# zjsun1017/CUDA-Go-ICP

Measured on AMD Instinct MI355X. Metric: bnb_cube_bounds_per_s, higher is better.
Workload: dtype f32; 1 GPU; bunny_goicp.toml (BASELINE configs[1]): N=30379 source, M=35947 target, DT 300^3, subsample 1.0; dt_layout=bricked4x4x4, exchange=local min

## Files before the change

cuda-go-icp_amd/binding.py:

```python
import ctypes as C
import os
import subprocess

HERE = os.path.dirname(os.path.abspath(__file__))
_LIB = None

OK = 0
STATUS = {-1: "GOICP_ERR_INVALID", -2: "GOICP_ERR_IO", -3: "GOICP_ERR_CONFIG", -4: "GOICP_ERR_NO_DEVICE",
          -5: "GOICP_ERR_DEVICE", -6: "GOICP_ERR_INTERNAL", -7: "GOICP_ERR_TIMEOUT", -8: "GOICP_ERR_PEER"}
PATH_MAX = 1024


class GoicpError(RuntimeError):
    def __init__(self, code, msg):
        super().__init__("%s: %s" % (STATUS.get(code, str(code)), msg))
        self.code = code


class CConfig(C.Structure):
    _fields_ = [("mode", C.c_int32), ("trim", C.c_int32), ("subsample", C.c_float), ("mse_threshold", C.c_float),
                ("resize", C.c_float), ("target", C.c_char * PATH_MAX), ("source", C.c_char * PATH_MAX),
                ("output", C.c_char * PATH_MAX), ("visualization", C.c_char * PATH_MAX),
                ("viz_theta", C.c_float), ("viz_phi", C.c_float), ("viz_spin_after_finish", C.c_int32),
                ("rot_min", C.c_float * 3), ("rot_max", C.c_float * 3), ("rot_search_depth", C.c_int32),
                ("trans_min", C.c_float * 3), ("trans_max", C.c_float * 3), ("trans_search_depth", C.c_int32),
                ("description", C.c_char * PATH_MAX), ("has_rotation_range", C.c_int32), ("has_translation_range", C.c_int32)]


class CParams(C.Structure):
    _fields_ = [("dt_size", C.c_int32), ("dt_expand", C.c_double), ("mse_threshold", C.c_float),
                ("dt_layout", C.c_int32), ("device", C.c_int32), ("trans_batch", C.c_int32),
                ("wide_children", C.c_int32), ("icp_max_iter", C.c_int32), ("verbose", C.c_int32),
                ("morton_sort", C.c_int32), ("rot_batch", C.c_int32), ("kd_gpu_build", C.c_int32), ("trim_fraction", C.c_float),
                ("use_rot_range", C.c_int32), ("use_trans_range", C.c_int32), ("rot_min", C.c_float * 3), ("rot_max", C.c_float * 3),
                ("trans_min", C.c_float * 3), ("trans_max", C.c_float * 3), ("rot_search_depth", C.c_int32), ("trans_search_depth", C.c_int32),
                ("icp_fused", C.c_int32), ("bounds_fp16", C.c_int32), ("icp_nn_cache", C.c_int32), ("flow", C.c_int32), ("adaptive_k", C.c_int32), ("queue_cap", C.c_int32), ("device_queues", C.c_int32),
                ("lds_tiles", C.c_int32), ("tile_spread_vox", C.c_float), ("tile_min", C.c_int32), ("stale_widen", C.c_int32), ("ub_tiebreak", C.c_int32), ("icp_point_seed", C.c_int32), ("ub_share", C.c_float), ("twin_fusion", C.c_int32), ("sort_items", C.c_int32), ("stale_compact", C.c_int32), ("stream_priority", C.c_int32), ("lanes", C.c_int32), ("lane_min_searches", C.c_int32),
                ("bounds_order", C.c_int32), ("bounds_order_min_groups", C.c_int32), ("bounds_order_max_runs", C.c_int32), ("bounds_order_cell", C.c_float), ("bounds_order_reprobe", C.c_int32),
                ("bounds_balance", C.c_int32), ("bounds_balance_a", C.c_float)]


class CCube(C.Structure):
    _fields_ = [("tx", C.c_float), ("ty", C.c_float), ("tz", C.c_float), ("delta", C.c_float),
                ("coeff", C.c_float), ("rot", C.c_int32)]


class CCounters(C.Structure):
    _fields_ = [(n, C.c_int64) for n in ("rot_pops", "trans_pops", "cubes", "inner_calls", "icp_runs", "icp_iters",
                                         "bounds_launches", "queue_fallbacks", "tile_expansions", "lane_batches")]


class CResult(C.Structure):
    _fields_ = [("optR", C.c_float * 9), ("optT", C.c_float * 3), ("curR", C.c_float * 9), ("curT", C.c_float * 3),
                ("best_sse", C.c_float), ("finished", C.c_int32), ("counters", CCounters),
                ("dt_build_ms", C.c_double), ("register_ms", C.c_double)]


class CStepStatus(C.Structure):
    _fields_ = [("finished", C.c_int32), ("early_exit", C.c_int32), ("best_sse", C.c_float),
                ("frontier_lb", C.c_float), ("rot_pops", C.c_int64)]


ALLREDUCE_FN = C.CFUNCTYPE(C.c_int, C.c_void_p, C.POINTER(C.c_uint64), C.c_size_t)
BCAST_FN = C.CFUNCTYPE(C.c_int, C.c_void_p, C.c_void_p, C.c_size_t, C.c_int32)


class CCommOps(C.Structure):
    _fields_ = [("ctx", C.c_void_p), ("rank", C.c_int32), ("world", C.c_int32), ("allreduce_min_u64", ALLREDUCE_FN), ("bcast", BCAST_FN)]


class CShardStats(C.Structure):
    _fields_ = [(n, C.c_int64) for n in ("steps", "exchanges", "broadcasts", "donations", "donated_cubes", "steps_idle")] + \
               [("wait_ms", C.c_double), ("step_ms", C.c_double), ("best_sse", C.c_float), ("failed_rank", C.c_int32)]


class CIcpShardStats(C.Structure):
    _fields_ = [(n, C.c_int32) for n in ("rank", "world", "block_begin", "block_end", "blocks", "sliced")] + \
               [(n, C.c_int64) for n in ("queries", "runs", "passes", "collectives")] + \
               [("sum_wait_ms", C.c_double), ("round_trip_ms", C.c_double)]


class CIcpOptions(C.Structure):
    _fields_ = [("metric", C.c_int32), ("normal_k", C.c_int32)]


class CIcpGate(C.Structure):
    _fields_ = [("max_corr_dist", C.c_float), ("min_inliers", C.c_int32), ("capped_walk", C.c_int32)]


class CIcpRobust(C.Structure):
    _fields_ = [("kernel", C.c_int32), ("scale", C.c_float)]


class CSourceFilter(C.Structure):
    _fields_ = [("voxel", C.c_float), ("radius", C.c_float), ("min_neighbors", C.c_int32)]


class CSourcePipeline(C.Structure):
    _fields_ = [("voxel", C.c_float), ("stat_neighbors", C.c_int32), ("stat_std_ratio", C.c_float), ("radius", C.c_float), ("min_neighbors", C.c_int32)]


class CClusterSelect(C.Structure):
    _fields_ = [("radius", C.c_float), ("min_neighbors", C.c_int32), ("min_size", C.c_int32), ("max_clusters", C.c_int32)]


class CPlaneSelect(C.Structure):
    _fields_ = [("distance", C.c_float), ("iterations", C.c_int32), ("refine", C.c_int32), ("max_planes", C.c_int32), ("min_inliers", C.c_int32),
                ("seed", C.c_uint64)]


class CPlane(C.Structure):
    _fields_ = [("normal", C.c_float * 3), ("point", C.c_float * 3), ("d", C.c_float), ("inliers", C.c_int32), ("hypothesis", C.c_int32),
                ("refined", C.c_int32)]


PLANE_MAX_ITERATIONS = 65536
PLANE_MAX_PLANES = 8


class CRansacPoseSelect(C.Structure):
    _fields_ = [("distance", C.c_float), ("iterations", C.c_int32), ("refine", C.c_int32), ("max_poses", C.c_int32), ("min_inliers", C.c_int32),
                ("edge_similarity", C.c_float), ("seed", C.c_uint64)]


class CRansacPose(C.Structure):
    _fields_ = [("R", C.c_float * 9), ("t", C.c_float * 3), ("inliers", C.c_int32), ("hypothesis", C.c_int32), ("refined", C.c_int32)]


RANSAC_POSE_MAX_ITERATIONS = 1 << 20
RANSAC_POSE_MAX_POSES = 64


class CPoseInfoOptions(C.Structure):
    _fields_ = [("metric", C.c_int32), ("use_pivot", C.c_int32), ("pivot", C.c_double * 3), ("rank_tol", C.c_double)]


class CPoseInfo(C.Structure):
    _fields_ = [("information", C.c_double * 36), ("gradient", C.c_double * 6), ("covariance", C.c_double * 36), ("eigenvalues", C.c_double * 6),
                ("eigenvectors", C.c_double * 36), ("pivot", C.c_double * 3), ("weight_sum", C.c_double), ("cost", C.c_double), ("sse", C.c_double),
                ("sigma2", C.c_double), ("inliers", C.c_int64), ("rank", C.c_int32), ("metric", C.c_int32), ("dof_nonpositive", C.c_int32)]


class CShardOptions(C.Structure):
    _fields_ = [("rot_pops_per_step", C.c_int32), ("rebalance", C.c_int32), ("stale_exchange", C.c_int32), ("ramp_to", C.c_int32)]


_fpp = C.POINTER(C.c_float)
ENG_BEGIN_FN = C.CFUNCTYPE(C.c_int, C.c_void_p, C.c_int32, C.c_int32)
ENG_STEP_FN = C.CFUNCTYPE(C.c_int, C.c_void_p, C.c_int32, C.POINTER(CStepStatus))
ENG_POSE_FN = C.CFUNCTYPE(C.c_int, C.c_void_p, _fpp, _fpp, _fpp)
ENG_OFFER_FN = C.CFUNCTYPE(C.c_int, C.c_void_p, C.c_float, _fpp, _fpp)
ENG_QSIZE_FN = C.CFUNCTYPE(C.c_int, C.c_void_p, C.POINTER(C.c_int32))
ENG_DONATE_FN = C.CFUNCTYPE(C.c_int, C.c_void_p, C.c_int32, _fpp, C.POINTER(C.c_int32))
ENG_RECEIVE_FN = C.CFUNCTYPE(C.c_int, C.c_void_p, _fpp, C.c_int32)
ENG_END_FN = C.CFUNCTYPE(C.c_int, C.c_void_p)


class CShardEngineOps(C.Structure):
    _fields_ = [("ctx", C.c_void_p), ("sse_threshold", C.c_float), ("begin", ENG_BEGIN_FN), ("step", ENG_STEP_FN), ("pose", ENG_POSE_FN),
                ("offer", ENG_OFFER_FN), ("queue_size", ENG_QSIZE_FN), ("donate", ENG_DONATE_FN), ("receive", ENG_RECEIVE_FN), ("end", ENG_END_FN)]


_fp, _vp = C.POINTER(C.c_float), C.c_void_p
SYMBOLS = {
    "goicp_last_error": (C.c_char_p, []),
    "goicp_abi_version": (C.c_int, []),
    "goicp_kernel_source_hash": (C.c_char_p, []),
    "goicp_config_load": (C.c_int, [C.c_char_p, C.POINTER(CConfig)]),
    "goicp_cloud_load": (C.c_int, [C.c_char_p, C.c_float, C.c_float, C.c_uint64, C.POINTER(_fp), C.POINTER(C.c_size_t)]),
    "goicp_cloud_free": (None, [_fp]),
    "goicp_params_default": (None, [C.POINTER(CParams)]),
    "goicp_params_from_config": (None, [C.POINTER(CConfig), C.POINTER(CParams)]),
    "goicp_thresholds": (C.c_int, [_vp, _fp, C.POINTER(C.c_int32)]),
    "goicp_device": (C.c_int, [_vp, C.POINTER(C.c_int32)]),
    "goicp_set_progress_callback": (C.c_int, [_vp, C.c_void_p, C.c_void_p]),
    "goicp_probe_gather": (C.c_int, [_vp, C.c_int32, C.c_size_t, C.POINTER(C.c_double)]),
    "goicp_debug_kabsch": (C.c_int, [_fp, _fp]),
    "goicp_debug_queue_expand": (C.c_int, [C.c_void_p, _fp, C.c_int32, _fp, C.c_int32, _fp, _fp, _fp, _fp, C.POINTER(C.c_int32)]),
    "goicp_debug_queue_expand_tiles": (C.c_int, [C.c_void_p, _fp, C.c_int32, _fp, C.c_int32, C.c_int32, _fp, _fp, _fp, _fp, C.POINTER(C.c_int32), C.c_int32, _fp,
                                                 C.POINTER(C.c_int32), _fp, _fp]),
    "goicp_debug_bounds_tile": (C.c_int, [C.c_void_p, _fp, _fp, C.c_int32, C.c_int32, C.c_int32, C.c_int32, _fp, _fp, _fp, _fp, _fp, C.POINTER(C.c_uint32)]),
    "goicp_debug_cache_hits": (C.c_int, [_vp, _fp, _fp, C.POINTER(C.c_int64)]),
    "goicp_debug_bounds_order": (C.c_int, [_vp, C.POINTER(C.c_int32)]),
    "goicp_debug_bounds_twins": (C.c_int, [_vp, C.POINTER(C.c_int32)]),
    "goicp_debug_bounds_balance": (C.c_int, [_vp, C.POINTER(C.c_int32)]),
    "goicp_debug_bounds_xcd_spans": (C.c_int, [_vp, C.POINTER(C.c_uint64)]),
    "goicp_debug_select": (C.c_int, [_vp, _fp, C.c_size_t, C.c_int32, C.c_int32, C.POINTER(C.c_uint8)]),
    "goicp_create": (C.c_int, [C.POINTER(CParams), _fp, C.c_size_t, _fp, C.c_size_t, C.POINTER(_vp)]),
    "goicp_destroy": (C.c_int, [_vp]),
    "goicp_dt_info": (C.c_int, [_vp, C.POINTER(C.c_int32), C.POINTER(C.c_double), C.POINTER(C.c_double)]),
    "goicp_dt_download": (C.c_int, [_vp, _fp]),
    "goicp_eval_bounds": (C.c_int, [_vp, _fp, _fp, C.c_size_t, C.c_int32, _fp, _fp]),
    "goicp_eval_bounds_batch": (C.c_int, [_vp, _fp, C.c_size_t, C.POINTER(CCube), C.c_size_t, _fp, _fp]),
    "goicp_eval_bounds_device": (C.c_int, [_vp, _vp, _vp, C.c_size_t, _vp, _vp, _vp]),
    "goicp_eval_bounds_device_grouped": (C.c_int, [_vp, _vp, C.c_size_t, _vp, C.c_size_t, _vp, _vp, _vp]),
    "goicp_time_bounds_device_grouped": (C.c_int, [_vp, _vp, C.c_size_t, _vp, C.c_size_t, _vp, _vp, C.c_int32, _fp]),
    "goicp_reduce_min_device": (C.c_int, [_vp, _vp, C.c_size_t, _vp, _vp, _vp]),
    "goicp_time_bounds_device": (C.c_int, [_vp, _vp, _vp, C.c_size_t, _vp, _vp, C.c_int32, _fp]),
    "goicp_rot_coeff": (C.c_float, [_vp, C.c_int32]),
    "goicp_trans_delta": (C.c_float, [C.c_float]),
    "goicp_rodrigues": (None, [_fp, _fp]),
    "goicp_eval_sse": (C.c_int, [_vp, _fp, _fp, _fp]),
    "goicp_inner_bnb": (C.c_int, [_vp, _fp, C.c_int32, C.c_float, _fp, _fp, C.POINTER(CCounters)]),
    "goicp_icp_run": (C.c_int, [_vp, _fp, _fp, C.c_int32, C.c_float, _fp, C.POINTER(C.c_int32)]),
    "goicp_icp_run_batch": (C.c_int, [_vp, C.c_size_t, _fp, _fp, C.c_int32, C.c_float, _fp, C.POINTER(C.c_int32)]),
    "goicp_time_icp_pass": (C.c_int, [_vp, _fp, _fp, C.c_int32, _fp]),
    "goicp_time_icp_pass_cached": (C.c_int, [_vp, _fp, _fp, C.c_int32, _fp]),
    "goicp_nn_query": (C.c_int, [_vp, _fp, C.c_size_t, C.POINTER(C.c_int32), _fp]),
    "goicp_icp_step": (C.c_int, [_vp]),
    "goicp_icp_options_default": (None, [C.POINTER(CIcpOptions)]),
    "goicp_set_icp_options": (C.c_int, [_vp, C.POINTER(CIcpOptions)]),
    "goicp_knn_query": (C.c_int, [_vp, _fp, C.c_size_t, C.c_int32, C.POINTER(C.c_int32), _fp]),
    "goicp_target_normals": (C.c_int, [_vp, _fp]),
    "goicp_set_icp_symmetric": (C.c_int, [_vp, C.c_int32, C.c_int32]),
    "goicp_get_icp_symmetric": (C.c_int, [_vp, C.POINTER(C.c_int32), C.POINTER(C.c_int32), C.POINTER(C.c_int32)]),
    "goicp_set_icp_generalized": (C.c_int, [_vp, C.c_int32, C.c_float, C.c_int32]),
    "goicp_get_icp_generalized": (C.c_int, [_vp, C.POINTER(C.c_int32), C.POINTER(C.c_float), C.POINTER(C.c_int32), C.POINTER(C.c_int32)]),
    "goicp_source_normals": (C.c_int, [_vp, _fp]),
    "goicp_set_source_normals": (C.c_int, [_vp, _fp, C.c_size_t]),
    "goicp_icp_gate_default": (None, [C.POINTER(CIcpGate)]),
    "goicp_set_icp_gate": (C.c_int, [_vp, C.POINTER(CIcpGate)]),
    "goicp_icp_inliers": (C.c_int, [_vp, C.c_size_t, C.POINTER(C.c_int32)]),
    "goicp_eval_correspondences": (C.c_int, [_vp, _fp, _fp, C.c_float, C.POINTER(C.c_int32), _fp, C.POINTER(C.c_int32), _fp]),
    "goicp_icp_robust_default": (None, [C.POINTER(CIcpRobust)]),
    "goicp_set_icp_robust": (C.c_int, [_vp, C.POINTER(CIcpRobust)]),
    "goicp_icp_robust_stats": (C.c_int, [_vp, C.c_size_t, _fp, _fp]),
    "goicp_pose_info_options_default": (None, [C.POINTER(CPoseInfoOptions)]),
    "goicp_pose_information": (C.c_int, [_vp, _fp, _fp, C.POINTER(CPoseInfoOptions), C.POINTER(CPoseInfo)]),
    "goicp_pose_information_batch": (C.c_int, [_vp, C.c_size_t, _fp, _fp, C.POINTER(CPoseInfoOptions), C.POINTER(CPoseInfo)]),
    "goicp_result_information": (C.c_int, [_vp, C.POINTER(CPoseInfoOptions), C.POINTER(CPoseInfo)]),
    "goicp_information_decompose": (C.c_int, [C.POINTER(C.c_double), C.c_double, C.POINTER(C.c_double), C.POINTER(C.c_double), C.POINTER(C.c_double), C.POINTER(C.c_int32)]),
    "goicp_set_search_truncation": (C.c_int, [_vp, C.c_float]),
    "goicp_set_source": (C.c_int, [_vp, _fp, C.c_size_t]),
    "goicp_source_order_host": (C.c_int, [_fp, C.c_size_t, C.c_int32, C.POINTER(C.c_int32)]),
    "goicp_debug_source_order": (C.c_int, [_vp, _fp, C.c_size_t, C.c_int32, C.POINTER(C.c_int32)]),
    "goicp_voxel_downsample_host": (C.c_int, [_fp, C.c_size_t, C.c_float, _fp, C.POINTER(C.c_int32), C.POINTER(C.c_size_t)]),
    "goicp_voxel_downsample": (C.c_int, [_vp, _fp, C.c_size_t, C.c_float, _fp, C.POINTER(C.c_int32), C.POINTER(C.c_size_t)]),
    "goicp_set_source_voxel": (C.c_int, [_vp, _fp, C.c_size_t, C.c_float, C.POINTER(C.c_size_t)]),
    "goicp_radius_outlier_removal_host": (C.c_int, [_fp, C.c_size_t, C.c_float, C.c_int32, _fp, C.POINTER(C.c_int32), C.POINTER(C.c_int32),
                                                   C.POINTER(C.c_size_t)]),
    "goicp_radius_outlier_removal": (C.c_int, [_vp, _fp, C.c_size_t, C.c_float, C.c_int32, _fp, C.POINTER(C.c_int32), C.POINTER(C.c_int32),
                                              C.POINTER(C.c_size_t)]),
    "goicp_source_filter_default": (None, [C.POINTER(CSourceFilter)]),
    "goicp_set_source_filtered": (C.c_int, [_vp, _fp, C.c_size_t, C.POINTER(CSourceFilter), C.POINTER(C.c_size_t)]),
    "goicp_statistical_outlier_removal_host": (C.c_int, [_fp, C.c_size_t, C.c_int32, C.c_float, _fp, C.POINTER(C.c_int32), _fp, C.POINTER(C.c_double),
                                                        C.POINTER(C.c_size_t)]),
    "goicp_statistical_outlier_removal": (C.c_int, [_vp, _fp, C.c_size_t, C.c_int32, C.c_float, _fp, C.POINTER(C.c_int32), _fp, C.POINTER(C.c_double),
                                                   C.POINTER(C.c_size_t)]),
    "goicp_source_pipeline_default": (None, [C.POINTER(CSourcePipeline)]),
    "goicp_set_source_pipeline": (C.c_int, [_vp, _fp, C.c_size_t, C.POINTER(CSourcePipeline), C.POINTER(C.c_size_t)]),
    "goicp_cluster_host": (C.c_int, [_fp, C.c_size_t, C.c_float, C.c_int32, C.POINTER(C.c_int32), C.POINTER(C.c_int32), C.POINTER(C.c_size_t)]),
    "goicp_cluster": (C.c_int, [_vp, _fp, C.c_size_t, C.c_float, C.c_int32, C.POINTER(C.c_int32), C.POINTER(C.c_int32), C.POINTER(C.c_size_t)]),
    "goicp_cluster_select_default": (None, [C.POINTER(CClusterSelect)]),
    "goicp_cluster_filter_host": (C.c_int, [_fp, C.c_size_t, C.POINTER(CClusterSelect), _fp, C.POINTER(C.c_int32), C.POINTER(C.c_int32),
                                           C.POINTER(C.c_size_t)]),
    "goicp_cluster_filter": (C.c_int, [_vp, _fp, C.c_size_t, C.POINTER(CClusterSelect), _fp, C.POINTER(C.c_int32), C.POINTER(C.c_int32),
                                      C.POINTER(C.c_size_t)]),
    "goicp_set_source_clustered": (C.c_int, [_vp, _fp, C.c_size_t, C.POINTER(CSourcePipeline), C.POINTER(CClusterSelect), C.POINTER(C.c_size_t)]),
    "goicp_plane_select_default": (None, [C.POINTER(CPlaneSelect)]),
    "goicp_segment_plane_host": (C.c_int, [_fp, C.c_size_t, C.POINTER(CPlaneSelect), C.POINTER(C.c_int32), C.POINTER(CPlane), C.POINTER(C.c_size_t)]),
    "goicp_segment_plane": (C.c_int, [_vp, _fp, C.c_size_t, C.POINTER(CPlaneSelect), C.POINTER(C.c_int32), C.POINTER(CPlane), C.POINTER(C.c_size_t)]),
    "goicp_plane_filter_host": (C.c_int, [_fp, C.c_size_t, C.POINTER(CPlaneSelect), _fp, C.POINTER(C.c_int32), C.POINTER(CPlane), C.POINTER(C.c_size_t),
                                         C.POINTER(C.c_size_t)]),
    "goicp_plane_filter": (C.c_int, [_vp, _fp, C.c_size_t, C.POINTER(CPlaneSelect), _fp, C.POINTER(C.c_int32), C.POINTER(CPlane), C.POINTER(C.c_size_t),
                                    C.POINTER(C.c_size_t)]),
    "goicp_set_source_segmented": (C.c_int, [_vp, _fp, C.c_size_t, C.POINTER(CSourcePipeline), C.POINTER(CPlaneSelect), C.POINTER(CClusterSelect),
                                            C.POINTER(C.c_size_t)]),
# ... 81 lines not shown
```

cuda-go-icp_amd/csrc/device.hip:

```cpp
#include <hip/hip_runtime.h>
#include <hip/hip_fp16.h>
#include <algorithm>
#include <climits>
#include <cstdlib>
#include <cmath>

#include "device.hpp"

namespace goicp {

__device__ __forceinline__ float wave_sum(float v)
{
#pragma unroll
	for (int off = 32; off > 0; off >>= 1) v += __shfl_xor(v, off, 64);
	return v;
}

__device__ __forceinline__ int xcd_remap(int bid, int nb)
{
	int q = nb >> 3, r = nb & 7, xcd = bid & 7;
	return (xcd < r ? xcd * (q + 1) : r * (q + 1) + (xcd - r) * q) + (bid >> 3);
}

__device__ __forceinline__ float half_bits_to_float(unsigned short h)
// ... 694 lines not shown
					if (worst <= eps_box) {
#pragma unroll
						for (int k = 0; k < 2; k++) {
							ix[k] = voxel_exact(qx[k], dt.xmin, dt.scale);
							iy[k] = voxel_exact(qy[k], dt.ymin, dt.scale);
							iz[k] = voxel_exact(qz[k], dt.zmin, dt.scale);
						}
					}
					const int ax[2] = {4 * ix[0] + cxyz, 4 * ix[1] + cxyz};
					const int ay[2] = {__mul24(iy[0], sy), __mul24(iy[1], sy)};
					const int az[2] = {__mul24(iz[0], sz), __mul24(iz[1], sz)};
					const float rho = coeff * q.w;
					const f2 rho2 = f2{rho, rho};
#pragma unroll
					for (int k = 0; k < 4; k++) {
						f2 v = f2{*reinterpret_cast<const float*>(tb + add3(ax[0], ay[k & 1], az[k >> 1])), *reinterpret_cast<const float*>(tb + add3(ax[1], ay[k & 1], az[k >> 1]))};
						f2 m = v;
						if constexpr (TRUNC) {
							if constexpr (!UB_PASS) v = v - rho2;
							m = trunc_clamp2(v, dt.trunc);
							ub2[k] = ub2[k] + m * m;
							const f2 dis = trunc_clamp2(v + ndelta2, dt.trunc);
							lb2[k] = lb2[k] + dis * dis;
						} else {
						if constexpr (!UB_PASS) {
							v = v - rho2;
							m = __builtin_elementwise_max(v, f2{0.f, 0.f});
						}
						ub2[k] = ub2[k] + m * m;
						const f2 dis = __builtin_elementwise_max(v + ndelta2, f2{0.f, 0.f});
						lb2[k] = lb2[k] + dis * dis;
						}
					}
				}
				};
				if (__builtin_amdgcn_readfirstlane(__float_as_int(coeff)) == 0 && coeff == 0.f) patch_points(std::true_type{});
				else patch_points(std::false_type{});
			} else {
				for (int j = wave + 4 * sub; j < np; j += 4 * L) {
					const float4 q = rp[j];
					float m[kGroup];
					sibling_residuals_rotated<1>(dt, q, ts, coeff * q.w, m);
#pragma unroll
					for (int k = 0; k < 4; k++) {
						const f2 m2 = f2{m[2 * k], m[2 * k + 1]};
						if constexpr (TRUNC) {
							const f2 mu = trunc_clamp2(m2, dt.trunc), dis = trunc_clamp2(m2 - delta2, dt.trunc);
							ub2[k] = ub2[k] + mu * mu;
							lb2[k] = lb2[k] + dis * dis;
						} else {
						ub2[k] = ub2[k] + m2 * m2;
						const f2 dis = __builtin_elementwise_max(m2 - delta2, f2{0.f, 0.f});
						lb2[k] = lb2[k] + dis * dis;
						}
					}
				}
			}
		}
		__syncthreads();
	}
	for (int off = P; off < 64; off <<= 1) {
#pragma unroll
		for (int k = 0; k < 4; k++) {
			ub2[k].x += __shfl_xor(ub2[k].x, off, 64); ub2[k].y += __shfl_xor(ub2[k].y, off, 64);
			lb2[k].x += __shfl_xor(lb2[k].x, off, 64); lb2[k].y += __shfl_xor(lb2[k].y, off, 64);
		}
	}
#pragma unroll
	for (int k = 0; k < 4; k++) {
		wacc[wave][lane][2 * k] = ub2[k].x; wacc[wave][lane][2 * k + 1] = ub2[k].y;
		wacc[wave][lane][kGroup + 2 * k] = lb2[k].x; wacc[wave][lane][kGroup + 2 * k + 1] = lb2[k].y;
	}
	__syncthreads();
	for (int idx = threadIdx.x; idx < sg.n * 2 * kGroup; idx += 256) {
		const int e = idx >> 4, k = idx & 15;
		const float s = ((wacc[0][e][k] + wacc[1][e][k]) + wacc[2][e][k]) + wacc[3][e][k];
		const int group = sg.off + e;
		if (chunks == 1) (k < kGroup ? ub_out : lb_out)[group * kGroup + (k & (kGroup - 1))] = s;
		else scratch[((size_t)group * chunks + chunk) * (2 * kGroup) + k] = s;
	}
	}
}

__global__ void bounds_finalize(const float* __restrict__ scratch, int B, int groups, int chunks, float* __restrict__ ub_out, float* __restrict__ lb_out);
hipError_t launch_bounds_tile(const float4* src, int N, const DtDesc& dt, const Rot9* rots, const ParentRec* parents, const void* segs, int nseg, int n,
                              int chunks, float* scratch, float* ub, float* lb, unsigned* stats, hipStream_t stream)
{
	if (dt.layout != 1 || n < 1 || n > 64 || nseg < 1 || chunks < 1) return hipErrorInvalidValue;
	int cp = (N + chunks - 1) / chunks;
	cp = (cp + kTilePatch - 1) / kTilePatch * kTilePatch;
	hipLaunchKernelGGL((dt.trunc > 0.f ? bounds_tile_kernel<false, true> : bounds_tile_kernel<false>), dim3(nseg * chunks), dim3(256), 0, stream, src, N, dt, rots, parents,
	                   static_cast<const TileSeg*>(segs), nseg, chunks, cp, static_cast<const int*>(nullptr), static_cast<int*>(nullptr), scratch, ub, lb, stats);
	if (chunks > 1) {
		const int groups = nseg * n, t = groups * 2 * kGroup;
		hipLaunchKernelGGL(bounds_finalize, dim3((t + 255) / 256), dim3(256), 0, stream, scratch, groups * kGroup, groups, chunks, ub, lb);
	}
	return hipGetLastError();
}

static inline bool bounds_lean(const DtDesc& dt) { return (size_t)dt.V * dt.V * dt.V * sizeof(float) <= ((size_t)256 << 20); }
bool bounds_uses_lean(const DtDesc& dt) { return dt.layout == 1 && bounds_lean(dt); }
constexpr int kTileQueueGrid = 256 * (160 * 1024 / (kTileFloats * 4 + 2048));
int bounds_tile_queue_grid() { return kTileQueueGrid; }
size_t bounds_tile_queue_scratch_floats(int max_groups)
{
	return (size_t)64 * ((size_t)kTileQueueGrid + (size_t)max_groups) * 2 * kGroup;
}
hipError_t launch_bounds_tile_queue(const float4* src, int N, const DtDesc& dt, const Rot9* rots, const QTile& tile, QCtl* ctl, int parity, hipStream_t stream)
{
	if (dt.layout != 1 || N <= 0) return hipErrorInvalidValue;
	hipLaunchKernelGGL((dt.trunc > 0.f ? bounds_tile_kernel<true, true> : bounds_tile_kernel<true>), dim3(kTileQueueGrid), dim3(256), 0, stream, src, N, dt, rots, tile.parents[parity], tile.segs[parity], 0, 1, 0,
	                   &ctl->n_tile_segs[parity], &ctl->tile_chunks, tile.scratch, tile.ub, tile.lb, static_cast<unsigned*>(nullptr));
	return hipGetLastError();
}

constexpr int kGroupCellBits = 4;
__device__ __forceinline__ unsigned cube_bucket(const CubeRec& c, int nrots)
{
	unsigned m = 0;
	const float t[3] = {c.tx, c.ty, c.tz};
#pragma unroll
	for (int k = 0; k < 3; k++) {
		const int q = min(max((int)((t[k] + 0.5f) * (float)(1 << kGroupCellBits)), 0), (1 << kGroupCellBits) - 1);
#pragma unroll
		for (int b = 0; b < kGroupCellBits; b++) m |= (unsigned)((q >> b) & 1) << (3 * b + k);
	}
	const unsigned rot = (unsigned)min(max(c.rot, 0), nrots - 1);
	return ((rot * 2u + (c.coeff > 0.f ? 1u : 0u)) << (3 * kGroupCellBits)) | m;
}
__global__ void cube_hist_kernel(const CubeRec* __restrict__ cubes, int B, int nrots, unsigned* __restrict__ hist)
{
	const int i = blockIdx.x * blockDim.x + threadIdx.x;
	if (i < B) atomicAdd(&hist[cube_bucket(cubes[i], nrots)], 1u);
}
__global__ __launch_bounds__(1024) void cube_scan_kernel(unsigned* __restrict__ hist, int nbins)
{
	__shared__ unsigned wtot[16];
	const int per = (nbins + 1023) / 1024, b0 = threadIdx.x * per;
	unsigned local = 0;
	for (int k = 0; k < per; k++) if (b0 + k < nbins) local += hist[b0 + k];
	unsigned incl = local;
#pragma unroll
	for (int o = 1; o < 64; o <<= 1) { const unsigned v = __shfl_up(incl, o, 64); if ((int)(threadIdx.x & 63) >= o) incl += v; }
	if ((threadIdx.x & 63) == 63) wtot[threadIdx.x >> 6] = incl;
	__syncthreads();
	unsigned before = 0;
	for (int w = 0; w < (int)(threadIdx.x >> 6); w++) before += wtot[w];
	unsigned run = before + incl - local;
	for (int k = 0; k < per; k++) if (b0 + k < nbins) { const unsigned c = hist[b0 + k]; hist[b0 + k] = run; run += c; }
}
__global__ void cube_scatter_kernel(const CubeRec* __restrict__ cubes, int B, int nrots, unsigned* __restrict__ offs, CubeRec* __restrict__ sorted, int* __restrict__ perm)
{
	const int i = blockIdx.x * blockDim.x + threadIdx.x;
	if (i >= B) return;
	const CubeRec c = cubes[i];
	const unsigned pos = atomicAdd(&offs[cube_bucket(c, nrots)], 1u);
	sorted[pos] = c;
	perm[pos] = i;
}
__global__ void cube_unpermute_kernel(const float* __restrict__ ub_s, const float* __restrict__ lb_s, const int* __restrict__ perm, int B, float* __restrict__ ub,
                                      float* __restrict__ lb)
{
	const int i = blockIdx.x * blockDim.x + threadIdx.x;
	if (i >= B) return;
	const int o = perm[i];
	ub[o] = ub_s[i]; lb[o] = lb_s[i];
}
size_t bounds_grouped_scratch_bytes(int B, int nrots)
{
	const size_t nbins = (size_t)nrots * 2 << (3 * kGroupCellBits);
	return sizeof(unsigned) * nbins + (sizeof(CubeRec) + sizeof(int) + 2 * sizeof(float)) * (size_t)B + 256;
}
hipError_t launch_bounds_grouped(const float4* src, int N, const DtDesc& dt, const Rot9* rots, int nrots, const CubeRec* cubes, int B, void* group_scratch,
                                 float* scratch, float* ub, float* lb, hipStream_t stream)
{
	if (B <= 0 || N <= 0) return hipSuccess;
	const int nbins = (nrots * 2) << (3 * kGroupCellBits);
	if (nrots < 1 || nbins > 1024 * 64) return hipErrorInvalidValue;
	char* p = static_cast<char*>(group_scratch);
	unsigned* hist = reinterpret_cast<unsigned*>(p); p += sizeof(unsigned) * (size_t)nbins;
	p = reinterpret_cast<char*>(((uintptr_t)p + 63) & ~(uintptr_t)63);
	CubeRec* sorted = reinterpret_cast<CubeRec*>(p); p += sizeof(CubeRec) * (size_t)B;
	int* perm = reinterpret_cast<int*>(p); p += sizeof(int) * (size_t)B;
	float* ub_s = reinterpret_cast<float*>(p); p += sizeof(float) * (size_t)B;
	float* lb_s = reinterpret_cast<float*>(p);
	hipError_t e = hipMemsetAsync(hist, 0, sizeof(unsigned) * (size_t)nbins, stream);
	if (e != hipSuccess) return e;
	const dim3 g((B + 255) / 256), b(256);
	hipLaunchKernelGGL(cube_hist_kernel, g, b, 0, stream, cubes, B, nrots, hist);
	hipLaunchKernelGGL(cube_scan_kernel, dim3(1), dim3(1024), 0, stream, hist, nbins);
	hipLaunchKernelGGL(cube_scatter_kernel, g, b, 0, stream, cubes, B, nrots, hist, sorted, perm);
	e = launch_bounds(src, N, dt, rots, sorted, nullptr, B, scratch, ub_s, lb_s, stream);
	if (e != hipSuccess) return e;
	hipLaunchKernelGGL(cube_unpermute_kernel, g, b, 0, stream, ub_s, lb_s, perm, B, ub, lb);
	return hipGetLastError();
}

template <int LAYOUT, bool LEAN = false, bool TRUNC = false>
__global__ __launch_bounds__(kBoundsThreads) void bounds_kernel(
    const float4* __restrict__ src, int N, DtDesc dt, const Rot9* __restrict__ rots,
    const CubeRec* __restrict__ cubes, const ParentRec* __restrict__ parents, int B, int groups, int chunks, int chunk_pts,
    float* __restrict__ scratch, float* __restrict__ ub_out, float* __restrict__ lb_out)
{
	__shared__ float red[kBoundsThreads / 64][2 * kGroup];
	bounds_work<LAYOUT, LEAN, TRUNC>(blockIdx.x, gridDim.x, src, N, dt, rots, cubes, parents, B, groups, chunks, chunk_pts, scratch, ub_out, lb_out, red);
}

__device__ __forceinline__ int group_rot(const CubeRec* __restrict__ cubes, int g) { return cubes[(size_t)g * kGroup].rot; }
__device__ __forceinline__ void group_centre(const CubeRec* __restrict__ cubes, int g, int B, float (&c)[3])
{
	const int i0 = g * kGroup, i1 = min(i0 + kGroup - 1, B - 1);
	const CubeRec a = cubes[i0], b = cubes[i1];
	c[0] = 0.5f * (a.tx + b.tx); c[1] = 0.5f * (a.ty + b.ty); c[2] = 0.5f * (a.tz + b.tz);
}
__device__ __forceinline__ void bounds_item_of(int work, int total, int groups, int chunks, int& group, int& chunk)
{
	if ((chunks & 7) == 0) {
		const int cpx = chunks >> 3, xcd = work & 7, slot = work >> 3;
		group = slot / cpx;
		chunk = xcd * cpx + (slot - group * cpx);
	} else {
		const int swz = xcd_remap(work, total);
		chunk = swz / groups; group = swz - chunk * groups;
	}
}
__device__ __forceinline__ int bounds_work_of(int group, int chunk, int groups, int chunks)
{
	if ((chunks & 7) == 0) {
		const int cpx = chunks >> 3, xcd = chunk / cpx;
		return ((group * cpx + (chunk - xcd * cpx)) << 3) | xcd;
	}
	const int nb = groups * chunks, q = nb >> 3, r = nb & 7, swz = chunk * groups + group;
	int xcd, off;
	if (swz < r * (q + 1)) { xcd = swz / (q + 1); off = swz - xcd * (q + 1); }
	else { const int t = swz - r * (q + 1); xcd = r + t / q; off = t - (xcd - r) * q; }
	return (off << 3) | xcd;
}
__device__ __forceinline__ unsigned order_key(const float (&c)[3], const float (&lo)[3], float to_cell)
{
	unsigned key = 0;
#pragma unroll
	for (int k = 0; k < 3; k++) {
		const unsigned v = (unsigned)min(max((int)((c[k] - lo[k]) * to_cell), 0), 31);
#pragma unroll
		for (int b = 0; b < 5; b++) key |= ((v >> b) & 1u) << (3 * b + k);
	}
	return key;
}
constexpr int kOrderHeld = 4;
__device__ __forceinline__ void bounds_cuts_store(const BoundsOrder& bo, int balanced, int items, int lane)
{
	const int x = min(lane, 8);
	int cut = balanced ? bounds_cut_of(bo.cost + kBoundsCost, x, items) : x * items;
	if (balanced) {
		const int cap = (int)(((long long)items * 5 + 3) / 4);
		for (int k = 1; k < 8; k++) { const int prev = __shfl(cut, k - 1, 64); if (lane == k) cut = min(cut, prev + cap); }
		for (int k = 7; k >= 1; k--) { const int next = __shfl(cut, k + 1, 64); if (lane == k) cut = max(cut, next - cap); }
	}
	if (lane <= 8) bo.ctl[kBoundsCut + lane] = cut;
}
__global__ __launch_bounds__(1024) void bounds_order_kernel(const CubeRec* __restrict__ cubes, int B, int G, DtDesc dt, BoundsOrder bo, int balanced)
{
	constexpr int per = kSortBins / 1024;
	constexpr int words = kSortBins + kSortBins / per;
	__shared__ __attribute__((aligned(16))) unsigned lds[words];
	__shared__ unsigned wtot[16];
	__shared__ int run_start[kBoundsOrderMaxRuns + 2];
	__shared__ int bound[kBoundsOrderMaxRuns];
	__shared__ int nbound;
	__shared__ float ext[16][6];
	const int tid = threadIdx.x, lane = tid & 63, wave = tid >> 6;
	static_assert(words % 4 == 0, "the counters are cleared four at a time");
	for (int i = tid; i < words / 4; i += 1024) reinterpret_cast<uint4*>(lds)[i] = make_uint4(0u, 0u, 0u, 0u);
	if (tid == 0) nbound = 0;
	__syncthreads();
	for (int base = 0; base < G; base += 8 * 1024) {
		int r[8], p[8];
#pragma unroll
		for (int k = 0; k < 8; k++) {
			const int g = min(base + k * 1024 + tid, G - 1);
			r[k] = group_rot(cubes, g);
			p[k] = lane == 0 ? group_rot(cubes, g > 0 ? g - 1 : 0) : 0;
		}
#pragma unroll
		for (int k = 0; k < 8; k++) {
			const int g = base + k * 1024 + tid, up = __shfl_up(r[k], 1, 64);
			if (lane) p[k] = up;
			if (g < G && r[k] != p[k]) { const int slot = atomicAdd(&nbound, 1); if (slot < kBoundsOrderMaxRuns) bound[slot] = g; }
		}
	}
	__syncthreads();
	const int nb = nbound, runs = nb + 1;
	if (runs > bo.max_runs) {
		if (blockIdx.x == 0 && tid == 0) {
			bo.ctl[0] = 0; bo.ctl[1] = 0; bo.ctl[2] = 0; bo.ctl[3] = 0; if (bo.host_note) *bo.host_note = ((long long)G << 1) | 1;
		}
		if (blockIdx.x == 0 && tid < 64) bounds_cuts_store(bo, balanced, (G + 1) >> 1, tid);
		return;
	}
	if (tid == 0) { run_start[0] = 0; run_start[runs] = G; }
	if (tid < nb) {
		const int b = bound[tid];
		int rank = 1;
		for (int q = 0; q < nb; q++) rank += (int)(bound[q] < b);
		run_start[rank] = b;
	}
	__syncthreads();
	const int run = blockIdx.x;
	if (run >= runs) return;
	const int s0 = run_start[run], n = run_start[run + 1] - s0;
	int item0 = 0, items = 0;
	for (int q = 0; q < runs; q++) { if (q == run) item0 = items; items += (run_start[q + 1] - run_start[q] + 1) >> 1; }
	if (run == 0 && tid == 0) { bo.ctl[0] = items; bo.ctl[1] = 1; bo.ctl[2] = 0; bo.ctl[3] = 0; if (bo.host_note) *bo.host_note = (long long)G << 1; }
	if (run == 0 && tid < 64) bounds_cuts_store(bo, balanced, items, tid);
	float held[kOrderHeld][3];
	float lo[3] = {INFINITY, INFINITY, INFINITY}, hi[3] = {-INFINITY, -INFINITY, -INFINITY};
#pragma unroll
	for (int h = 0; h < kOrderHeld; h++) group_centre(cubes, s0 + min(tid + h * 1024, n - 1), B, held[h]);
#pragma unroll
	for (int h = 0; h < kOrderHeld; h++) {
#pragma unroll
		for (int k = 0; k < 3; k++) { lo[k] = fminf(lo[k], held[h][k]); hi[k] = fmaxf(hi[k], held[h][k]); }
	}
	for (int j = tid + kOrderHeld * 1024; j < n; j += 1024) {
		float c[3];
		group_centre(cubes, s0 + j, B, c);
#pragma unroll
		for (int k = 0; k < 3; k++) { lo[k] = fminf(lo[k], c[k]); hi[k] = fmaxf(hi[k], c[k]); }
	}
#pragma unroll
	for (int k = 0; k < 3; k++) {
#pragma unroll
		for (int o = 32; o > 0; o >>= 1) { lo[k] = fminf(lo[k], __shfl_xor(lo[k], o, 64)); hi[k] = fmaxf(hi[k], __shfl_xor(hi[k], o, 64)); }
		if (lane == 0) { ext[wave][k] = lo[k]; ext[wave][3 + k] = hi[k]; }
	}
	__syncthreads();
	float span = 0.f;
#pragma unroll
	for (int k = 0; k < 3; k++) {
		for (int w = 0; w < 16; w++) { lo[k] = fminf(lo[k], ext[w][k]); hi[k] = fmaxf(hi[k], ext[w][3 + k]); }
		span = fmaxf(span, hi[k] - lo[k]);
	}
	const float cell = fmaxf(fmaxf(bo.cell_vox, 1.f), span * dt.scale_f * (1.f / 31.5f));
	const float to_cell = dt.scale_f / cell;
	unsigned key[kOrderHeld];
#pragma unroll
	for (int h = 0; h < kOrderHeld; h++) {
		key[h] = order_key(held[h], lo, to_cell);
		if (tid + h * 1024 < n) atomicAdd(&lds[key[h] + key[h] / per], 1u);
	}
	for (int j = tid + kOrderHeld * 1024; j < n; j += 1024) {
		float c[3];
		group_centre(cubes, s0 + j, B, c);
		const unsigned kj = order_key(c, lo, to_cell);
		atomicAdd(&lds[kj + kj / per], 1u);
	}
	__syncthreads();
	const int b0 = tid * (per + 1);
	unsigned local = 0;
#pragma unroll
	for (int k = 0; k < per; k++) local += lds[b0 + k];
	unsigned incl = local;
#pragma unroll
	for (int o = 1; o < 64; o <<= 1) { const unsigned v = __shfl_up(incl, o, 64); if (lane >= o) incl += v; }
	if (lane == 63) wtot[wave] = incl;
	__syncthreads();
	unsigned before = 0;
	for (int w = 0; w < wave; w++) before += wtot[w];
	unsigned runsum = before + incl - local;
#pragma unroll
	for (int k = 0; k < per; k++) { const unsigned c = lds[b0 + k]; lds[b0 + k] = runsum; runsum += c; }
	__syncthreads();
	auto place = [&](unsigned kj, int j) {
		const int pos = (int)atomicAdd(&lds[kj + kj / per], 1u), it = item0 + (pos >> 1);
		bo.order[s0 + pos] = (unsigned)(s0 + j);
		bo.pairs[2 * it + (pos & 1)] = s0 + j;
		if (pos == n - 1 && !(pos & 1)) bo.pairs[2 * it + 1] = -1;
	};
#pragma unroll
	for (int h = 0; h < kOrderHeld; h++)
		if (tid + h * 1024 < n) place(key[h], tid + h * 1024);
	for (int j = tid + kOrderHeld * 1024; j < n; j += 1024) {
		float c[3];
		group_centre(cubes, s0 + j, B, c);
		place(order_key(c, lo, to_cell), j);
	}
}

template <bool TRUNC>
__global__ __launch_bounds__(kBoundsThreads) void bounds_ordered_kernel(
    const float4* __restrict__ src, int N, DtDesc dt, const Rot9* __restrict__ rots,
    const CubeRec* __restrict__ cubes, const ParentRec* __restrict__ parents, int B, int groups, int chunks, int chunk_pts,
    float* __restrict__ scratch, float* __restrict__ ub_out, float* __restrict__ lb_out, const unsigned* __restrict__ order, const int* __restrict__ ctl, int gate)
{
	__shared__ float red[kBoundsThreads / 64][2 * kGroup];
	int work = blockIdx.x;
	if (ctl[1]) {
		if (!gate) return;
		int group, chunk;
		bounds_item_of(work, gridDim.x, groups, chunks, group, chunk);
		work = bounds_work_of((int)order[group], chunk, groups, chunks);
	}
	bounds_work<1, true, TRUNC>(work, gridDim.x, src, N, dt, rots, cubes, parents, B, groups, chunks, chunk_pts, scratch, ub_out, lb_out, red);
}

__device__ __forceinline__ bool pair_member(const CubeRec* __restrict__ cubes, const ParentRec* __restrict__ parents, int group, int B, PairMember& m, int& rot)
{
	CubeRec cr[kGroup];
	load_group(cubes, parents, group, B, cr);
	bool sib = group * kGroup + kGroup <= B;
#pragma unroll
	for (int c = 0; c < kGroup; c++)
		sib = sib && cr[c].rot == cr[0].rot && cr[c].tx == cr[c & 1].tx && cr[c].ty == cr[c & 2].ty && cr[c].tz == cr[c & 4].tz &&
		      cr[c].delta == cr[0].delta && cr[c].coeff == cr[0].coeff;
	m.ts = SiblingSet{cr[0].tx, cr[1].tx, cr[0].ty, cr[2].ty, cr[0].tz, cr[4].tz};
	m.delta = cr[0].delta; m.coeff = cr[0].coeff; rot = cr[0].rot;
	return sib;
}
__device__ __forceinline__ bool same_box(const PairMember& a, const PairMember& b)
{
	const unsigned d = (__float_as_uint(a.ts.tx0) ^ __float_as_uint(b.ts.tx0)) | (__float_as_uint(a.ts.tx1) ^ __float_as_uint(b.ts.tx1)) |
	                   (__float_as_uint(a.ts.ty0) ^ __float_as_uint(b.ts.ty0)) | (__float_as_uint(a.ts.ty1) ^ __float_as_uint(b.ts.ty1)) |
	                   (__float_as_uint(a.ts.tz0) ^ __float_as_uint(b.ts.tz0)) | (__float_as_uint(a.ts.tz1) ^ __float_as_uint(b.ts.tz1)) |
	                   (__float_as_uint(a.delta) ^ __float_as_uint(b.delta));
	return d == 0u;
}
#ifdef GOICP_BOUNDS_XCD_STAMPS
#define GOICP_BOUNDS_PAIR_HEAD __device__ __forceinline__ void bounds_pair_body
#else
#define GOICP_BOUNDS_PAIR_HEAD __global__ __launch_bounds__(kBoundsThreads) void bounds_pair_kernel
#endif
template <bool TRUNC>
GOICP_BOUNDS_PAIR_HEAD(
    const float4* __restrict__ src, int N, DtDesc dt, const Rot9* __restrict__ rots,
    const CubeRec* __restrict__ cubes, const ParentRec* __restrict__ parents, int B, int groups, int max_items, int chunks, int chunk_pts,
    float* __restrict__ scratch, float* __restrict__ ub_out, float* __restrict__ lb_out, const int* __restrict__ pairs, int* __restrict__ ctl)
{
	__shared__ float red[kBoundsThreads / 64][2 * kGroup];
	const int work = blockIdx.x, total = gridDim.x;
	int chunk, item;
	if (chunks == 8) {
		const int xcd = work & 7, u = ctl[kBoundsCut + xcd] + (work >> 3);
		if (u >= ctl[kBoundsCut + xcd + 1]) return;
		const int items = ctl[kBoundsCut + 8] >> 3;
		chunk = u / items;
		item = u - chunk * items;
	} else if ((chunks & 7) == 0) {
		const int cpx = chunks >> 3, xcd = work & 7, slot = work >> 3;
		item = slot / cpx;
		chunk = xcd * cpx + (slot - item * cpx);
	} else {
		const int swz = xcd_remap(work, total);
		chunk = swz / max_items; item = swz - chunk * max_items;
	}
	const bool listed = ctl[1] != 0;
	int ga, gb;
	if (listed) {
		if (item >= ctl[0]) return;
		ga = pairs[2 * item]; gb = pairs[2 * item + 1];
	} else {
		ga = 2 * item;
		if (ga >= groups) return;
		gb = ga + 1 < groups ? ga + 1 : -1;
	}
	if (listed && gb >= 0) {
		PairMember A, Bm;
		int ra, rb;
		const bool sa = pair_member(cubes, parents, ga, B, A, ra), sb = pair_member(cubes, parents, gb, B, Bm, rb);
		if (sa && sb && ra == rb) {
			const Rot9 R0 = rots[ra];
			const int p0 = chunk * chunk_pts;
			const int p1 = p0 + chunk_pts < N ? p0 + chunk_pts : N;
			if (same_box(A, Bm)) {
				const bool same = __float_as_uint(A.coeff) == __float_as_uint(Bm.coeff) || (A.coeff == 0.f && Bm.coeff == 0.f);
				if (chunk == 0 && threadIdx.x == 0) atomicAdd(ctl + (same ? 3 : 2), 1);
				float ub[kGroup], lb[kGroup];
				if (same) {
					f2 ub2[1][4], lb2[1][4];
#pragma unroll
					for (int k = 0; k < 4; k++) { ub2[0][k] = f2{0.f, 0.f}; lb2[0][k] = f2{0.f, 0.f}; }
					const float co[1] = {A.coeff};
					if (A.coeff == 0.f) lean_points<1, 1, true, TRUNC>(src, p0, p1, dt, R0, A.ts, A.delta, co, ub2, lb2);
					else lean_points<1, 1, false, TRUNC>(src, p0, p1, dt, R0, A.ts, A.delta, co, ub2, lb2);
#pragma unroll
					for (int k = 0; k < 4; k++) { ub[2 * k] = ub2[0][k].x; ub[2 * k + 1] = ub2[0][k].y; lb[2 * k] = lb2[0][k].x; lb[2 * k + 1] = lb2[0][k].y; }
					bounds_item_store(ub, lb, ga, chunk, chunks, B, scratch, ub_out, lb_out, red, gb);
					return;
				}
				if (A.coeff == 0.f) {
					const float c = A.coeff; A.coeff = Bm.coeff; Bm.coeff = c;
					const int g = ga; ga = gb; gb = g;
				}
				f2 ub2[2][4], lb2[2][4];
#pragma unroll
				for (int q = 0; q < 2; q++)
#pragma unroll
					for (int k = 0; k < 4; k++) { ub2[q][k] = f2{0.f, 0.f}; lb2[q][k] = f2{0.f, 0.f}; }
				const float co[2] = {A.coeff, Bm.coeff};
				if (Bm.coeff == 0.f) lean_points<1, 2, true, TRUNC>(src, p0, p1, dt, R0, A.ts, A.delta, co, ub2, lb2);
				else lean_points<1, 2, false, TRUNC>(src, p0, p1, dt, R0, A.ts, A.delta, co, ub2, lb2);
#pragma unroll
				for (int k = 0; k < 4; k++) { ub[2 * k] = ub2[1][k].x; ub[2 * k + 1] = ub2[1][k].y; lb[2 * k] = lb2[1][k].x; lb[2 * k + 1] = lb2[1][k].y; }
				bounds_item_store(ub, lb, gb, chunk, chunks, B, scratch, ub_out, lb_out, red);
				__syncthreads();
#pragma unroll
				for (int k = 0; k < 4; k++) { ub[2 * k] = ub2[0][k].x; ub[2 * k + 1] = ub2[0][k].y; lb[2 * k] = lb2[0][k].x; lb[2 * k + 1] = lb2[0][k].y; }
				bounds_item_store(ub, lb, ga, chunk, chunks, B, scratch, ub_out, lb_out, red);
				return;
			}
			if (A.coeff != 0.f && Bm.coeff == 0.f) {
				const PairMember t = A; A = Bm; Bm = t;
				const int g = ga; ga = gb; gb = g;
			}
			f2 ubA[4], lbA[4], ubB[4], lbB[4];
#pragma unroll
			for (int k = 0; k < 4; k++) { ubA[k] = f2{0.f, 0.f}; lbA[k] = f2{0.f, 0.f}; ubB[k] = f2{0.f, 0.f}; lbB[k] = f2{0.f, 0.f}; }
			bool okA = true, okB = true;
			if (A.coeff == 0.f && Bm.coeff == 0.f) lean_points_pair<true, true, TRUNC>(src, p0, p1, dt, R0, A, Bm, ubA, lbA, ubB, lbB, okA, okB);
			else if (A.coeff == 0.f) lean_points_pair<true, false, TRUNC>(src, p0, p1, dt, R0, A, Bm, ubA, lbA, ubB, lbB, okA, okB);
			else lean_points_pair<false, false, TRUNC>(src, p0, p1, dt, R0, A, Bm, ubA, lbA, ubB, lbB, okA, okB);
			const int bad = (__syncthreads_or(okA ? 0 : 1) ? 1 : 0) | (__syncthreads_or(okB ? 0 : 1) ? 2 : 0);
			float ub[kGroup], lb[kGroup];
			if (!(bad & 1)) {
#pragma unroll
				for (int k = 0; k < 4; k++) { ub[2 * k] = ubA[k].x; ub[2 * k + 1] = ubA[k].y; lb[2 * k] = lbA[k].x; lb[2 * k + 1] = lbA[k].y; }
				bounds_item_store(ub, lb, ga, chunk, chunks, B, scratch, ub_out, lb_out, red);
				__syncthreads();
			}
			if (!(bad & 2)) {
#pragma unroll
				for (int k = 0; k < 4; k++) { ub[2 * k] = ubB[k].x; ub[2 * k + 1] = ubB[k].y; lb[2 * k] = lbB[k].x; lb[2 * k + 1] = lbB[k].y; }
				bounds_item_store(ub, lb, gb, chunk, chunks, B, scratch, ub_out, lb_out, red);
				__syncthreads();
			}
			if (bad == 0) return;
			if (!(bad & 1)) ga = gb;
			if (bad != 3) gb = -1;
		}
	}
#pragma unroll 1
	for (int m = 0; m < 2; m++) {
		const int g = m ? gb : ga;
		if (g < 0) break;
		if (m) __syncthreads();
		bounds_work<1, true, TRUNC>(bounds_work_of(g, chunk, groups, chunks), groups * chunks, src, N, dt, rots, cubes, parents, B, groups, chunks, chunk_pts, scratch, ub_out, lb_out, red);
	}
}
#undef GOICP_BOUNDS_PAIR_HEAD
#ifdef GOICP_BOUNDS_XCD_STAMPS
constexpr int kXcdStampStride = 16;
__device__ unsigned long long g_xcd_stamps[kXcdStampRows * kXcdStampStride];
template <bool TRUNC>
__global__ __launch_bounds__(kBoundsThreads) void bounds_pair_kernel(
    const float4* __restrict__ src, int N, DtDesc dt, const Rot9* __restrict__ rots,
    const CubeRec* __restrict__ cubes, const ParentRec* __restrict__ parents, int B, int groups, int max_items, int chunks, int chunk_pts,
    float* __restrict__ scratch, float* __restrict__ ub_out, float* __restrict__ lb_out, const int* __restrict__ pairs, int* __restrict__ ctl)
{
	const unsigned long long t0 = wall_clock64();
	bounds_pair_body<TRUNC>(src, N, dt, rots, cubes, parents, B, groups, max_items, chunks, chunk_pts, scratch, ub_out, lb_out, pairs, ctl);
	__syncthreads();
	if (threadIdx.x == 0) {
		const unsigned long long t1 = wall_clock64();
		const unsigned xcc = __builtin_amdgcn_s_getreg(20 | (3 << 11)) & 7u;
		const unsigned rows[2] = {xcc, 8u + (blockIdx.x & 7u)};
		for (int k = 0; k < 2; k++) {
			unsigned long long* s = g_xcd_stamps + rows[k] * kXcdStampStride;
			if (t1 - t0 < 100ull) { atomicAdd(s + 5, 1ull); continue; }
			atomicMin(s + 0, t0); atomicMax(s + 1, t1); atomicAdd(s + 2, 1ull); atomicAdd(s + 3, t1 - t0);
		}
		atomicOr(g_xcd_stamps + xcc * kXcdStampStride + 4, 1ull << (blockIdx.x & 7u));
	}
}
#endif

__host__ __device__ inline void bounds_shape(int B, int N, int* groups, int* chunks, int* chunk_pts);
template <int LAYOUT, bool LEAN = false, bool TRUNC = false>
__global__ __launch_bounds__(kBoundsThreads) void bounds_queue_kernel(
    const float4* __restrict__ src, int N, DtDesc dt, const Rot9* __restrict__ rots, const ParentRec* __restrict__ parents,
    const int* __restrict__ d_groups, int* __restrict__ work8, int* __restrict__ d_chunks, float* __restrict__ scratch, float* __restrict__ ub_out,
    float* __restrict__ lb_out, const QSearch* __restrict__ searches, const int* __restrict__ parent_search, QSort qs)
{
	__shared__ float red[kBoundsThreads / 64][2 * kGroup];
	__shared__ int next_item[2];
	__shared__ int twin_sh;
	const TwinCtx twin{LEAN ? searches : nullptr, parent_search, &twin_sh};
	const int ngroups = *d_groups;
	if (ngroups <= 0) return;
	int groups, chunks, chunk_pts;
	const bool sorted = qsort_on(qs, ngroups);
	if (sorted) { groups = ngroups; chunks = qs.chunks; chunk_pts = qs.chunk_pts; }
	else bounds_shape(ngroups * kGroup, N, &groups, &chunks, &chunk_pts);
	if (blockIdx.x == 0 && threadIdx.x == 0) *d_chunks = chunks;
	if (sorted)
		for (int i = blockIdx.x * kBoundsThreads + threadIdx.x; i < kSortBins; i += gridDim.x * kBoundsThreads) qs.hist[i] = 0u;
	const int total = groups * chunks;
	const bool per_xcd = sorted || (total & 7) == 0;
	const int slot = per_xcd ? (int)(blockIdx.x & 7) : 0, stride = per_xcd ? 8 : 1;
	int* ctr = work8 + slot;
	if (threadIdx.x == 0) next_item[0] = atomicAdd(ctr, 1);
	__syncthreads();
	int item = next_item[0], buf = 0;
	while (item * stride + slot < total) {
		if (threadIdx.x == 0) next_item[buf ^ 1] = atomicAdd(ctr, 1);
		bounds_work<LAYOUT, LEAN, TRUNC>(item * stride + slot, total, src, N, dt, rots, nullptr, parents, ngroups * kGroup, groups, chunks, chunk_pts, scratch, ub_out,
		                    lb_out, red, sorted ? qs.order : nullptr, twin);
		__syncthreads();
		buf ^= 1;
		item = next_item[buf];
	}
}

__global__ void bounds_finalize(const float* __restrict__ scratch, int B, int groups, int chunks,
                                float* __restrict__ ub_out, float* __restrict__ lb_out)
{
	int t = blockIdx.x * blockDim.x + threadIdx.x;
	if (t >= groups * 2 * kGroup) return;
	int group = t / (2 * kGroup), k = t - group * 2 * kGroup;
	int c = group * kGroup + (k & (kGroup - 1));
	if (c >= B) return;
	const float* s = scratch + (size_t)group * chunks * (2 * kGroup) + k;
	float acc = 0.f;
	for (int j = 0; j < chunks; j++) acc += s[(size_t)j * 2 * kGroup];
	(k < kGroup ? ub_out : lb_out)[c] = acc;
}

constexpr int kTrimThreads = 1024;
template <int LAYOUT>
__global__ __launch_bounds__(kTrimThreads) void bounds_trim_kernel(
    const float4* __restrict__ src, int N, DtDesc dt, const Rot9* __restrict__ rots,
    const CubeRec* __restrict__ cubes, const ParentRec* __restrict__ parents, int B, int inliers,
    float* __restrict__ ub_out, float* __restrict__ lb_out, const int* __restrict__ d_groups, int* __restrict__ d_chunks = nullptr)
{
	if (d_groups) {
		if (d_chunks && blockIdx.x == 0 && threadIdx.x == 0) *d_chunks = 1;
		if ((int)blockIdx.x >= *d_groups) return;
		B = *d_groups * kGroup;
	}
	__shared__ unsigned hist[kGroup][2048];
	__shared__ unsigned sel_prefix[kGroup], sel_rem[kGroup];
	__shared__ float red[kTrimThreads / 64][2 * kGroup];
	const int c0 = blockIdx.x * kGroup;
	CubeRec cr[kGroup];
	load_group(cubes, parents, blockIdx.x, B, cr);
	if (threadIdx.x < kGroup) { sel_prefix[threadIdx.x] = 0u; sel_rem[threadIdx.x] = (unsigned)inliers; }

	const bool sib = is_sibling_set(cr) && c0 + kGroup <= B;
	const Rot9 R0 = rots[cr[0].rot];
	const SiblingSet ts{cr[0].tx, cr[1].tx, cr[0].ty, cr[2].ty, cr[0].tz, cr[4].tz};
	auto residuals = [&](const float4& p, float m[kGroup]) {
		if (sib) { sibling_residuals<LAYOUT>(dt, R0, ts, p, cr[0].coeff * p.w, m); return; }
#pragma unroll
		for (int c = 0; c < kGroup; c++) {
			const Rot9 R = rots[cr[c].rot];
			const float rx = R.r[0] * p.x + R.r[1] * p.y + R.r[2] * p.z;
			const float ry = R.r[3] * p.x + R.r[4] * p.y + R.r[5] * p.z;
			const float rz = R.r[6] * p.x + R.r[7] * p.y + R.r[8] * p.z;
			float v = dt_distance<LAYOUT>(dt, rx + cr[c].tx, ry + cr[c].ty, rz + cr[c].tz);
			v = v - cr[c].coeff * p.w;
			m[c] = v < 0.f ? 0.f : v;
		}
	};

#pragma unroll 1
	for (int pass = 0; pass < 3; pass++) {
		const int shift = pass == 0 ? 20 : (pass == 1 ? 9 : 0), width = pass == 2 ? 9 : 11, bins = 1 << width;
		for (int i = threadIdx.x; i < kGroup * 2048; i += kTrimThreads) (&hist[0][0])[i] = 0u;
		__syncthreads();
		for (int i = threadIdx.x; i < N; i += kTrimThreads) {
			const float4 p = src[i];
			float m[kGroup];
			residuals(p, m);
#pragma unroll
			for (int c = 0; c < kGroup; c++) {
				const unsigned key = __float_as_uint(m[c]);
				if (pass == 0 || (key >> (shift + width)) == sel_prefix[c])
					atomicAdd(&hist[c][(key >> shift) & (unsigned)(bins - 1)], 1u);
			}
		}
		__syncthreads();
		if (threadIdx.x < 32 * kGroup) {
			const int c = threadIdx.x >> 5, j = threadIdx.x & 31, per = bins >> 5;
			unsigned local = 0;
			for (int b = j * per; b < (j + 1) * per; b++) local += hist[c][b];
			unsigned incl = local;
#pragma unroll
			for (int off = 1; off < 32; off <<= 1) {
				const unsigned o = __shfl_up(incl, off, 32);
				if (j >= off) incl += o;
			}
			const unsigned excl = incl - local, rem = sel_rem[c];
			if (excl < rem && rem <= incl) {
				unsigned cum = excl;
				for (int b = j * per; b < (j + 1) * per; b++) {
					const unsigned h = hist[c][b];
					if (cum < rem && rem <= cum + h) {
						sel_prefix[c] = (sel_prefix[c] << width) | (unsigned)b;
						sel_rem[c] = rem - cum;
						break;
					}
					cum += h;
				}
			}
		}
// ... 191 lines not shown
	for (int i = threadIdx.x; i < kSortBins; i += 1024) qs.hist[i] = lds[i + i / per];
}
int qsort_shift(int V) { int s = 0; while (((V - 1) >> s) >= 32) s++; return s; }
size_t qsort_hist_bytes() { return sizeof(unsigned) * kSortBins; }
hipError_t launch_queue_sort(const ParentRec* parents, const Rot9* rots, const int* d_groups, int max_groups, const QSort& qs, const DtDesc& dt, hipStream_t stream)
{
	if (!qs.order || max_groups < qs.min_groups) return hipSuccess;
	const int blocks = (int)std::min<size_t>(((size_t)max_groups * qs.chunks + 255) / 256, 2048);
	hipLaunchKernelGGL(task_key_kernel, dim3(blocks), dim3(256), 0, stream, parents, rots, d_groups, qs, dt);
	hipLaunchKernelGGL(task_scan_kernel, dim3(1), dim3(1024), 0, stream, d_groups, qs);
	hipLaunchKernelGGL(task_scatter_kernel, dim3(blocks), dim3(256), 0, stream, d_groups, qs);
	return hipGetLastError();
}

__constant__ float kCostRots[4][9] = {
	{1.f, 0.f, 0.f, 0.f, 1.f, 0.f, 0.f, 0.f, 1.f},
	{0.84567982f, -0.449964464f, -0.286980212f, 0.0414698496f, 0.591505408f, -0.805233896f, 0.532076955f, 0.669069052f, 0.518884122f},
	{0.219921082f, -0.74321264f, 0.631877899f, 0.372148067f, 0.662668586f, 0.649904728f, -0.901743054f, 0.0922243893f, 0.422319949f},
	{0.122044131f, 0.98462534f, 0.124972485f, -0.646330416f, 0.174399301f, -0.742860556f, -0.753234506f, 0.00988825131f, 0.65767777f}};
__global__ __launch_bounds__(256) void bounds_chunk_cost_kernel(const float4* __restrict__ src, int N, int chunk_pts, DtDesc dt, int* __restrict__ cost)
{
	const int i = blockIdx.x * 256 + (int)threadIdx.x, lane = (int)threadIdx.x & 63, first_pt = i - lane;
	if (first_pt >= N) return;
	const bool have = i < N;
	const float4 p = src[have ? i : N - 1];
	const unsigned V = (unsigned)dt.V;
	int lines = 0;
	for (int r = 0; r < 4; r++) {
		const float* R = kCostRots[r];
		const float rx = R[0] * p.x + R[1] * p.y + R[2] * p.z, ry = R[3] * p.x + R[4] * p.y + R[5] * p.z, rz = R[6] * p.x + R[7] * p.y + R[8] * p.z;
		const int ix = (int)((rx - dt.xmin_f) * dt.scale_f + 0.5f), iy = (int)((ry - dt.ymin_f) * dt.scale_f + 0.5f), iz = (int)((rz - dt.zmin_f) * dt.scale_f + 0.5f);
		const bool in = have && (unsigned)ix < V && (unsigned)iy < V && (unsigned)iz < V;
		const int line = in ? (int)((((((unsigned)iz >> 2) * (unsigned)dt.VB + ((unsigned)iy >> 2)) * (unsigned)dt.VB + ((unsigned)ix >> 2)) << 1) | (((unsigned)iz >> 1) & 1u)) : -1;
		bool first = in;
		for (int j = 0; j < 63; j++) {
			const int o = __shfl(line, j, 64);
			if (j < lane && o == line) first = false;
		}
		lines += __popcll(__ballot(first));
	}
	if (lane == 0) { const int chunk = first_pt / chunk_pts; atomicAdd(cost + chunk, lines); atomicAdd(cost + 8 + chunk, 4); }
}
__global__ void bounds_cut_plan_kernel(int* __restrict__ cost, int a_q8)
{
	if (blockIdx.x == 0 && threadIdx.x == 0) bounds_cut_plan(cost, a_q8, cost + kBoundsCost);
}
hipError_t launch_bounds_chunk_cost(const float4* src, int N, const DtDesc& dt, int a_q8, int* cost, hipStream_t stream)
{
	hipError_t e = hipMemsetAsync(cost, 0, kBoundsCost * sizeof(int), stream);
	if (e != hipSuccess) return e;
	if ((N + kBoundsThreads - 1) / kBoundsThreads >= 32 && dt.layout == 1 && bounds_lean(dt)) {
		int chunk_pts = (N + 7) / 8;
		chunk_pts = (chunk_pts + kBoundsThreads - 1) / kBoundsThreads * kBoundsThreads;
		hipLaunchKernelGGL(bounds_chunk_cost_kernel, dim3((N + 255) / 256), dim3(256), 0, stream, src, N, chunk_pts, dt, cost);
	}
	hipLaunchKernelGGL(bounds_cut_plan_kernel, dim3(1), dim3(64), 0, stream, cost, a_q8);
	return hipGetLastError();
}

hipError_t bounds_xcd_stamps_take(unsigned long long* out, hipStream_t stream)
{
#ifdef GOICP_BOUNDS_XCD_STAMPS
	unsigned long long clear[kXcdStampRows * kXcdStampStride] = {}, got[kXcdStampRows * kXcdStampStride];
	for (int r = 0; r < kXcdStampRows; r++) clear[r * kXcdStampStride] = ~0ull;
	hipError_t e = hipStreamSynchronize(stream);
	if (e == hipSuccess) e = hipMemcpyFromSymbol(got, HIP_SYMBOL(g_xcd_stamps), sizeof(got));
	if (e == hipSuccess) e = hipMemcpyToSymbol(HIP_SYMBOL(g_xcd_stamps), clear, sizeof(clear));
	for (int r = 0; r < kXcdStampRows; r++)
		for (int c = 0; c < kXcdStampCols; c++) out[r * kXcdStampCols + c] = got[r * kXcdStampStride + c];
	return e;
#else
	(void)out; (void)stream;
	return hipErrorNotSupported;
#endif
}

hipError_t launch_bounds(const float4* src, int N, const DtDesc& dt, const Rot9* rots, const CubeRec* cubes, const ParentRec* parents,
                         int B, float* scratch, float* ub, float* lb, hipStream_t stream, const BoundsOrder* bo)
{
	if (B <= 0 || N <= 0) return hipSuccess;
	int groups, chunks, chunk_pts;
	bounds_shape(B, N, &groups, &chunks, &chunk_pts);
	dim3 grid(groups * chunks), block(kBoundsThreads);
	if (bo && bo->mode > 0 && cubes && !parents && dt.layout == 1 && bounds_lean(dt) && groups >= bo->min_groups && bo->max_runs >= 1 && bo->max_runs <= kBoundsOrderMaxRuns) {
		const bool balanced = bo->mode == 2 && chunks == 8 && bo->balance && bo->cost;
		hipLaunchKernelGGL(bounds_order_kernel, dim3(bo->max_runs), dim3(1024), 0, stream, cubes, B, groups, dt, *bo, balanced ? 1 : 0);
		if (bo->mode == 1) {
			hipLaunchKernelGGL((dt.trunc > 0.f ? bounds_ordered_kernel<true> : bounds_ordered_kernel<false>), grid, block, 0, stream, src, N, dt, rots, cubes, parents, B, groups,
			                   chunks, chunk_pts, scratch, ub, lb, bo->order, bo->ctl, 1);
		} else {
			const int max_items = (int)bounds_order_items(groups, bo->max_runs);
			const int nblocks = chunks == 8 ? 8 * bounds_pair_slots(max_items, balanced) : max_items * chunks;
			hipLaunchKernelGGL((dt.trunc > 0.f ? bounds_pair_kernel<true> : bounds_pair_kernel<false>), dim3(nblocks), block, 0, stream, src, N, dt, rots, cubes, parents,
			                   B, groups, max_items, chunks, chunk_pts, scratch, ub, lb, bo->pairs, bo->ctl);
		}
	} else
	if (dt.trunc > 0.f) {
		if (dt.layout == 0)
			hipLaunchKernelGGL((bounds_kernel<0, false, true>), grid, block, 0, stream, src, N, dt, rots, cubes, parents, B, groups, chunks, chunk_pts, scratch, ub, lb);
		else if (dt.layout == 1 && bounds_lean(dt))
			hipLaunchKernelGGL((bounds_kernel<1, true, true>), grid, block, 0, stream, src, N, dt, rots, cubes, parents, B, groups, chunks, chunk_pts, scratch, ub, lb);
		else if (dt.layout == 1)
			hipLaunchKernelGGL((bounds_kernel<1, false, true>), grid, block, 0, stream, src, N, dt, rots, cubes, parents, B, groups, chunks, chunk_pts, scratch, ub, lb);
		else
			hipLaunchKernelGGL((bounds_kernel<2, false, true>), grid, block, 0, stream, src, N, dt, rots, cubes, parents, B, groups, chunks, chunk_pts, scratch, ub, lb);
	} else
	if (dt.layout == 0)
		hipLaunchKernelGGL(bounds_kernel<0>, grid, block, 0, stream, src, N, dt, rots, cubes, parents, B, groups, chunks, chunk_pts, scratch, ub, lb);
	else if (dt.layout == 1 && bounds_lean(dt))
		hipLaunchKernelGGL((bounds_kernel<1, true>), grid, block, 0, stream, src, N, dt, rots, cubes, parents, B, groups, chunks, chunk_pts, scratch, ub, lb);
	else if (dt.layout == 1)
		hipLaunchKernelGGL(bounds_kernel<1>, grid, block, 0, stream, src, N, dt, rots, cubes, parents, B, groups, chunks, chunk_pts, scratch, ub, lb);
	else
		hipLaunchKernelGGL(bounds_kernel<2>, grid, block, 0, stream, src, N, dt, rots, cubes, parents, B, groups, chunks, chunk_pts, scratch, ub, lb);
	if (chunks > 1) {
		int t = groups * 2 * kGroup;
		hipLaunchKernelGGL(bounds_finalize, dim3((t + 255) / 256), dim3(256), 0, stream, scratch, B, groups, chunks, ub, lb);
	}
	return hipGetLastError();
}

#ifndef GOICP_ICP_THREADS
#define GOICP_ICP_THREADS 256
#endif
constexpr int kIcpThreads = GOICP_ICP_THREADS;

template <int LAYOUT>
__device__ __forceinline__ float nn_upper_bound(const DtDesc& dt, float qx, float qy, float qz)
{
	const float inv = 1.0f / dt.scale_f;
	const int V1 = dt.V - 1;
	const int ix = min(max((int)rintf((qx - dt.xmin_f) * dt.scale_f), 0), V1);
	const int iy = min(max((int)rintf((qy - dt.ymin_f) * dt.scale_f), 0), V1);
	const int iz = min(max((int)rintf((qz - dt.zmin_f) * dt.scale_f), 0), V1);
	const float cx = dt.xmin_f + (float)ix * inv, cy = dt.ymin_f + (float)iy * inv, cz = dt.zmin_f + (float)iz * inv;
	const float ex = qx - cx, ey = qy - cy, ez = qz - cz;
	const float d = (__fsqrt_rn(ex * ex + ey * ey + ez * ez) + dt_fetch<LAYOUT>(dt, ix, iy, iz) + 0.9f * inv) * 1.00001f;
	return d * d;
}

template <int CTRL>
__device__ __forceinline__ unsigned dpp_u32(unsigned v)
{
	return (unsigned)__builtin_amdgcn_update_dpp((int)v, (int)v, CTRL, 0xF, 0xF, false);
}
__device__ __forceinline__ unsigned row_min_u32(unsigned v)
{
	v = min(v, dpp_u32<0xB1>(v));
	v = min(v, dpp_u32<0x4E>(v));
	v = min(v, dpp_u32<0x141>(v));
	v = min(v, dpp_u32<0x140>(v));
	return v;
}

template <int CTRL>
__device__ __forceinline__ float dpp_f32(float v)
{
	return __int_as_float(__builtin_amdgcn_update_dpp(__float_as_int(v), __float_as_int(v), CTRL, 0xF, 0xF, false));
}
__device__ __forceinline__ float row_sum_f32(float v)
{
	v += dpp_f32<0xB1>(v);
	v += dpp_f32<0x4E>(v);
	v += dpp_f32<0x141>(v);
	v += dpp_f32<0x140>(v);
	return v;
}

struct Box6x4 { float4 lox, loy, loz, hix, hiy, hiz; };
__device__ __forceinline__ Box6x4 load_child_boxes4(const float* __restrict__ g, int l)
{
	const float4* r = reinterpret_cast<const float4*>(g);
	return Box6x4{r[l], r[16 + l], r[32 + l], r[48 + l], r[64 + l], r[80 + l]};
}
__device__ __forceinline__ float box_lb1(float lox, float loy, float loz, float hix, float hiy, float hiz, float qx, float qy, float qz)
{
	const float ex = fmaxf(fmaxf(lox - qx, qx - hix), 0.f);
	const float ey = fmaxf(fmaxf(loy - qy, qy - hiy), 0.f);
	const float ez = fmaxf(fmaxf(loz - qz, qz - hiz), 0.f);
	float d = ex * ex;
	d += ey * ey;
	d += ez * ez;
	return d;
}
__device__ __forceinline__ void boxes_lb4(const Box6x4& b, float qx, float qy, float qz, float lb[4])
{
	lb[0] = box_lb1(b.lox.x, b.loy.x, b.loz.x, b.hix.x, b.hiy.x, b.hiz.x, qx, qy, qz);
	lb[1] = box_lb1(b.lox.y, b.loy.y, b.loz.y, b.hix.y, b.hiy.y, b.hiz.y, qx, qy, qz);
	lb[2] = box_lb1(b.lox.z, b.loy.z, b.loz.z, b.hix.z, b.hiy.z, b.hiz.z, qx, qy, qz);
	lb[3] = box_lb1(b.lox.w, b.loy.w, b.loz.w, b.hix.w, b.hiy.w, b.hiz.w, qx, qy, qz);
}
__device__ __forceinline__ void boxes_keys4(const Box6x4& b, float qx, float qy, float qz, unsigned key[4])
{
	float lb[4];
	boxes_lb4(b, qx, qy, qz, lb);
#pragma unroll
	for (int j = 0; j < 4; j++) key[j] = (__float_as_uint(lb[j]) & ~3u) | (unsigned)j;
}
__device__ __forceinline__ unsigned row_take(unsigned key[4], int l, int row, int& child)
{
// ... 2366 lines not shown
```

cuda-go-icp_amd/csrc/device.hpp:

```cpp
#pragma once
#include <hip/hip_runtime_api.h>
#include <cmath>
#include <cstddef>
#include <cstdint>

#include "../../include/goicp_mi355.h"

namespace goicp {

#if defined(__HIPCC__)
__host__ __device__
#endif
inline bool cube_in_range(float x, float y, float z, float w, const float lo[3], const float hi[3])
{
	return x + w > lo[0] && x <= hi[0] && y + w > lo[1] && y <= hi[1] && z + w > lo[2] && z <= hi[2];
}

#if defined(__HIPCC__)
__host__ __device__
#endif
inline unsigned brick_x(unsigned x) { return x & 3u; }
#if defined(__HIPCC__)
__host__ __device__
#endif
inline unsigned brick_y(unsigned y) { return (y & 3u) << 2; }
#if defined(__HIPCC__)
__host__ __device__
#endif
inline unsigned brick_z(unsigned z) { return (z & 3u) << 4; }
#if defined(__HIPCC__)
__host__ __device__
#endif
inline size_t brick_index(size_t x, size_t y, size_t z, size_t VB)
{
	return (((z >> 2) * VB + (y >> 2)) * VB + (x >> 2)) * 64 + (brick_x((unsigned)x) | brick_y((unsigned)y) | brick_z((unsigned)z));
}

struct DtDesc {
	const float* grid;
	int V;
	int VB;
	int layout;
	float trunc;
	double scale;
	double xmin, ymin, zmin;
	float scale_f, xmin_f, ymin_f, zmin_f;
	float c1, c2;
	const double* overshoot;
	int n_overshoot;
	const int32_t* nn_ids;
};
static_assert(sizeof(DtDesc) == 104 && offsetof(DtDesc, trunc) == 20 && offsetof(DtDesc, scale) == 24, "DtDesc layout");

struct CubeRec {
	float tx, ty, tz;
	float delta;
	float coeff;
	int32_t rot;
};
static_assert(sizeof(CubeRec) == 24, "CubeRec layout");

struct ParentRec {
	float x, y, z;
	float w;
	float coeff;
	int32_t rot;
};
static_assert(sizeof(ParentRec) == 24, "ParentRec layout");

struct Rot9 { float r[9]; };

constexpr int kLeafSlots = 16;
constexpr int kMaxLevels = 3;
struct KdDesc {
	const float* boxes[kMaxLevels];
	const float4* pts;
	int K;
	int M;
};

struct Pose { float R[9]; float t[3]; };

constexpr int kGroup = 8;
constexpr int kBoundsThreads = 256;
constexpr int kIcpAcc = 16;
constexpr double kIcpRankTol = 1e-6;
constexpr double kIcpCovNoise = 0x1p-20;

size_t bounds_scratch_floats(int B, int N, int* groups_out, int* chunks_out);
struct BoundsOrder {
	int mode;
	int min_groups, max_runs;
	float cell_vox;
	unsigned* keys;
	unsigned* order;
	int* pairs;
	int* ctl;
	long long* host_note;
	const int* cost;
	int balance;
};
constexpr int kBoundsOrderMaxRuns = 64;
constexpr int kBoundsCut = 4, kBoundsCtlInts = 32;
constexpr float kBoundsBalanceA = 18.f;
inline size_t bounds_order_items(int groups, int max_runs) { return (size_t)(groups + 1) / 2 + (size_t)max_runs; }
inline int bounds_pair_slots(int max_items, bool balanced) { return balanced ? (int)(((long long)max_items * 5 + 3) / 4) : max_items; }
constexpr int kBoundsCost = 16, kBoundsPlan = 24;
#if defined(__HIPCC__)
__host__ __device__
#endif
inline void bounds_cut_plan(const int* cost, int a_q8, int plan[kBoundsPlan])
{
	long long w[8], sum = 0;
	for (int k = 0; k < 8; k++) { w[k] = (long long)a_q8 * cost[8 + k] + 256ll * cost[k]; sum += w[k]; }
	for (int x = 0; x < 8; x++) { plan[x] = x; plan[8 + x] = 0; plan[16 + x] = 1; }
	if (sum <= 0) return;
	while (sum >= (1ll << 39)) { sum = 0; for (int k = 0; k < 8; k++) { w[k] >>= 1; sum += w[k]; } }
	long long total = 0;
	for (int k = 0; k < 8; k++) {
		long long s = (w[k] << 23) / sum;
		s = s < 838861 ? 838861 : (s > 1310720 ? 1310720 : s);
		w[k] = s; total += s;
	}
	int k = 0;
	long long before = 0;
	for (int x = 1; x < 8; x++) {
		while (k < 7 && 8 * (before + w[k]) <= x * total) { before += w[k]; k++; }
		plan[x] = k; plan[8 + x] = (int)(x * total - 8 * before); plan[16 + x] = (int)(8 * w[k]);
	}
}
#if defined(__HIPCC__)
__host__ __device__
#endif
inline int bounds_cut_of(const int* plan, int x, int items)
{
	if (x <= 0) return 0;
	if (x >= 8) return 8 * items;
	const long long d = plan[16 + x];
	long long j = ((long long)items * plan[8 + x] + d - 1) / d;
	if (j > items) j = items;
	return (int)((long long)plan[x] * items + j);
}
#if defined(__HIPCC__)
__host__ __device__
#endif
inline void bounds_cut_cap(int cut[9], int items)
{
	const int cap = (int)(((long long)items * 5 + 3) / 4);
	for (int x = 1; x < 8; x++) if (cut[x] > cut[x - 1] + cap) cut[x] = cut[x - 1] + cap;
	for (int x = 7; x >= 1; x--) if (cut[x] < cut[x + 1] - cap) cut[x] = cut[x + 1] - cap;
}
inline void bounds_cuts(const int* cost, int a_q8, int items, int cut[9])
{
	int plan[kBoundsPlan];
	bounds_cut_plan(cost, a_q8, plan);
	for (int x = 0; x < 9; x++) cut[x] = bounds_cut_of(plan, x, items);
	bounds_cut_cap(cut, items);
}
hipError_t launch_bounds(const float4* src, int N, const DtDesc& dt, const Rot9* rots, const CubeRec* cubes, const ParentRec* parents,
                         int B, float* scratch, float* ub, float* lb, hipStream_t stream, const BoundsOrder* bo = nullptr);
hipError_t launch_bounds_chunk_cost(const float4* src, int N, const DtDesc& dt, int a_q8, int* cost, hipStream_t stream);
constexpr int kXcdStampRows = 16, kXcdStampCols = 6;
hipError_t bounds_xcd_stamps_take(unsigned long long* out, hipStream_t stream);

size_t bounds_grouped_scratch_bytes(int B, int nrots);
hipError_t launch_bounds_grouped(const float4* src, int N, const DtDesc& dt, const Rot9* rots, int nrots, const CubeRec* cubes, int B, void* group_scratch,
                                 float* scratch, float* ub, float* lb, hipStream_t stream);

hipError_t launch_bounds_trim(const float4* src, int N, const DtDesc& dt, const Rot9* rots, const CubeRec* cubes, const ParentRec* parents, int B,
                              int inliers, float* ub, float* lb, hipStream_t stream);

constexpr int kQueueCap = 8192;
constexpr int kQueueMaxPop = 512;
constexpr int kQueueRoundPop = 128;
struct QNode { float x, y, z, w, ub, lb; };
struct QSearch {
	float best;
	float coeff;
	int32_t rot;
	int32_t count;
	int32_t done, improved;
	int32_t n_parents, parent_off;
	int32_t pops, cubes;
	float bx, by, bz, bw;
	int32_t tile;
	float min_ub;
// ... 552 lines not shown
```

cuda-go-icp_amd/csrc/engine.cpp:

```cpp
#include "engine.hpp"
#include "comm.hpp"
#include "trace.hpp"

#include <algorithm>
#include <chrono>
#include <cmath>
#include <cstdio>
#include <cstdlib>
#include <cstring>
#include <limits>
#include <stdexcept>

namespace goicp {

namespace {

constexpr double kPI = 3.1415926536;
constexpr double kSQRT3 = 1.732050808;
constexpr int kMaxRotLevel = 20;

double now_ms()
{
	return std::chrono::duration<double, std::milli>(std::chrono::steady_clock::now().time_since_epoch()).count();
}
// ... 1093 lines not shown
	Buf<int32_t> d_perm(n);
	HIPCHK(launch_source_order(d_xyz, (int)n, mode, mn, ext, d_perm, stream_));
	HIPCHK(hipMemcpyAsync(perm, d_perm, sizeof(int32_t) * n, hipMemcpyDeviceToHost, stream_));
	HIPCHK(hipStreamSynchronize(stream_));
}

Engine::~Engine()
{
	if (!stream_) return;
	int prev = -1;
	if (hipGetDevice(&prev) == hipSuccess && prev != dev_) { hipSetDevice(dev_); restore_device_.prev = prev; }
	for (int k = 0; k < kMaxLanes; k++) if (lane_stream_[k]) hipStreamSynchronize(lane_stream_[k]);
}
Engine::RestoreDevice::~RestoreDevice() { if (prev >= 0) hipSetDevice(prev); }

void Engine::make_lane_stream(int li)
{
	lane_own_[li].create();
	lane_stream_[li] = lane_own_[li];
}

void Engine::ensure_batch(size_t B, size_t K)
{
	if (B > cap_cubes_) {
		size_t cap = std::max<size_t>(B, cap_cubes_ * 2);
		hipStreamSynchronize(stream_);
		cap_cubes_ = 0;
		d_cubes_.alloc(cap); d_ub_.alloc(cap); d_lb_.alloc(cap);
		h_cubes_.alloc(cap); h_ub_.alloc(cap); h_lb_.alloc(cap);
		cap_cubes_ = cap;
	}
	if (K > cap_rots_) {
		size_t cap = std::max<size_t>(K, cap_rots_ * 2);
		hipStreamSynchronize(stream_);
		cap_rots_ = 0;
		d_rots_.alloc(cap); h_rots_.alloc(cap);
		cap_rots_ = cap;
	}
	size_t need = bounds_scratch_floats((int)std::max<size_t>(B, 1), (int)N_, nullptr, nullptr);
	size_t worst = (size_t)2 * kGroup * (8 * ((cap_cubes_ + kGroup - 1) / kGroup) + 4096);
	need = std::max(need, worst);
	if (need > d_scratch_.size()) {
		hipStreamSynchronize(stream_);
		d_scratch_.alloc(need);
	}
}

void Engine::upload_rots(const std::vector<Rot9>& rots)
{
	ensure_batch(1, rots.size());
	std::memcpy(h_rots_, rots.data(), sizeof(Rot9) * rots.size());
	HIPCHK(hipMemcpyAsync(d_rots_, h_rots_, sizeof(Rot9) * rots.size(), hipMemcpyHostToDevice, stream_));
}

void Engine::ensure_bounds_scratch(int B, hipStream_t s)
{
	const size_t need = bounds_scratch_floats(B, (int)N_, nullptr, nullptr);
	if (need <= d_scratch_.size()) return;
	HIPCHK(hipStreamSynchronize(stream_));
	if (s && s != stream_) HIPCHK(hipStreamSynchronize(s));
	d_scratch_.alloc(need);
}

const BoundsOrder* Engine::ensure_bounds_order(int B, hipStream_t s)
{
	const int groups = (B + kGroup - 1) / kGroup;
	if (p_.bounds_order <= 0 || groups < p_.bounds_order_min_groups || !bounds_uses_lean(bounds_dt())) return nullptr;
	if (!h_border_note_) { h_border_note_.alloc(1); *h_border_note_.get() = -1; }
	if (p_.bounds_order_reprobe > 0) {
		const long long note = *static_cast<volatile long long*>(h_border_note_.get());
		if (note == (((long long)groups << 1) | 1) && ++border_skipped_ < p_.bounds_order_reprobe) return nullptr;
		border_skipped_ = 0;
	}
	const int max_runs = std::min(std::max(p_.bounds_order_max_runs, 1), kBoundsOrderMaxRuns);
	const size_t items = bounds_order_items(groups, max_runs), ctl_at = (2 * (size_t)groups + 2 * items + kBoundsCtlInts - 1) / kBoundsCtlInts * kBoundsCtlInts;
	const size_t need = ctl_at + kBoundsCtlInts;
	if (need > d_border_.size()) {
		HIPCHK(hipStreamSynchronize(stream_));
		if (s && s != stream_) HIPCHK(hipStreamSynchronize(s));
		d_border_.alloc(need + need / 2);
	}
	border_.mode = p_.bounds_order >= 2 ? 2 : 1;
	border_.min_groups = p_.bounds_order_min_groups; border_.max_runs = max_runs; border_.cell_vox = p_.bounds_order_cell;
	border_.keys = d_border_.get(); border_.order = border_.keys + groups;
	border_.pairs = reinterpret_cast<int*>(border_.order + groups); border_.ctl = reinterpret_cast<int*>(border_.keys + ctl_at);
	border_.host_note = h_border_note_.get();
	border_.cost = d_bcost_.get(); border_.balance = p_.bounds_balance != 0;
	return &border_;
}

void Engine::eval_bounds_dev(const Rot9* d_rots, const CubeRec* d_cubes, int B, float* d_ub, float* d_lb, hipStream_t s, const ParentRec* d_parents)
{
	DeviceGuard guard(dev_);
	ensure_bounds_scratch(B, s);
	if (inliers_ < (int)N_)
		HIPCHK(launch_bounds_trim(d_src_, (int)N_, dt_, d_rots, d_cubes, d_parents, B, inliers_, d_ub, d_lb, s ? s : stream_));
	else
	{
		const BoundsOrder* bo = d_cubes && !d_parents ? ensure_bounds_order(B, s) : nullptr;
		HIPCHK(launch_bounds(d_src_, (int)N_, bounds_dt(), d_rots, d_cubes, d_parents, B, d_scratch_, d_ub, d_lb, s ? s : stream_, bo));
		border_form_ = bo ? bo->mode : 0; border_stream_ = s ? s : stream_;
		int groups = 0;
		bounds_scratch_floats(B, (int)N_, &groups, &border_chunks_);
		border_items_ = (groups + 1) / 2;
	}
	cnt_.bounds_launches++;
}

void Engine::debug_bounds_order(int info[3])
{
	DeviceGuard guard(dev_);
	info[0] = border_form_; info[1] = info[2] = 0;
	if (!border_form_) return;
	int ctl[2] = {0, 0};
	HIPCHK(hipStreamSynchronize(border_stream_));
	HIPCHK(hipMemcpy(ctl, border_.ctl, sizeof(ctl), hipMemcpyDeviceToHost));
	info[1] = ctl[1]; info[2] = ctl[0];
}

void Engine::debug_bounds_twins(int info[2])
{
	DeviceGuard guard(dev_);
	info[0] = info[1] = 0;
	if (border_form_ != 2) return;
	HIPCHK(hipStreamSynchronize(border_stream_));
	HIPCHK(hipMemcpy(info, border_.ctl + 2, 2 * sizeof(int), hipMemcpyDeviceToHost));
}

void Engine::debug_bounds_balance(int info[26])
{
	DeviceGuard guard(dev_);
	for (int x = 0; x < 26; x++) info[x] = 0;
	HIPCHK(hipStreamSynchronize(stream_));
	if (d_bcost_) HIPCHK(hipMemcpy(info + 9, d_bcost_, 16 * sizeof(int), hipMemcpyDeviceToHost));
	if (border_form_ == 2 && border_chunks_ == 8) {
		HIPCHK(hipStreamSynchronize(border_stream_));
		HIPCHK(hipMemcpy(info, border_.ctl + kBoundsCut, 9 * sizeof(int), hipMemcpyDeviceToHost));
		info[25] = border_.balance && border_.cost ? 1 : 0;
	} else {
		int items = border_items_;
		if (border_form_) {
			int ctl[2] = {0, 0};
			HIPCHK(hipStreamSynchronize(border_stream_));
			HIPCHK(hipMemcpy(ctl, border_.ctl, sizeof(ctl), hipMemcpyDeviceToHost));
			if (ctl[1]) items = ctl[0];
		}
		for (int x = 0; x < 9; x++) info[x] = x * items;
	}
}

bool Engine::debug_bounds_xcd_spans(unsigned long long* out)
{
	DeviceGuard guard(dev_);
	const hipError_t e = bounds_xcd_stamps_take(out, border_stream_ ? border_stream_ : stream_);
	if (e == hipErrorNotSupported) return false;
	HIPCHK(e);
	return true;
}

void Engine::reduce_min_dev(const float* d_v, int n, float* d_min, int* d_idx, hipStream_t s)
{
	DeviceGuard guard(dev_);
	HIPCHK(launch_reduce_min(d_v, n, d_min, d_idx, s ? s : stream_));
}

void Engine::eval_bounds_dev_grouped(const Rot9* d_rots, int nrots, const CubeRec* d_cubes, int B, float* d_ub, float* d_lb, hipStream_t s)
{
	DeviceGuard guard(dev_);
	if (inliers_ < (int)N_) { eval_bounds_dev(d_rots, d_cubes, B, d_ub, d_lb, s); return; }
	if (nrots < 1 || nrots > 16) throw std::invalid_argument("goicp: grouped bounds take 1..16 rotations");
	ensure_bounds_scratch(B, s);
	void* gs = scratch_bytes(bounds_grouped_scratch_bytes(B, nrots));
	HIPCHK(launch_bounds_grouped(d_src_, (int)N_, bounds_dt(), d_rots, nrots, d_cubes, B, gs, d_scratch_, d_ub, d_lb, s ? s : stream_));
	cnt_.bounds_launches++;
}

float Engine::time_bounds_dev(const Rot9* d_rots, const CubeRec* d_cubes, int B, float* d_ub, float* d_lb, int iters, int grouped_nrots)
{
	DeviceGuard guard(dev_);
	auto once = [&] { if (grouped_nrots > 0) eval_bounds_dev_grouped(d_rots, grouped_nrots, d_cubes, B, d_ub, d_lb, stream_); else eval_bounds_dev(d_rots, d_cubes, B, d_ub, d_lb, stream_); };
	once();
	HIPCHK(hipStreamSynchronize(stream_));
	HIPCHK(hipEventRecord(ev0_, stream_));
	for (int i = 0; i < iters; i++) once();
	HIPCHK(hipEventRecord(ev1_, stream_));
	HIPCHK(hipEventSynchronize(ev1_));
	float ms = 0.f;
	HIPCHK(hipEventElapsedTime(&ms, ev0_, ev1_));
	return ms / (float)std::max(iters, 1);
}

void Engine::eval_bounds_batch(const float* rots9, size_t K, const CubeRec* cubes, size_t B, float* ub, float* lb)
{
	if (B == 0) return;
	DeviceGuard guard(dev_);
	for (size_t i = 0; i < B; i++)
		if (cubes[i].rot < 0 || (size_t)cubes[i].rot >= K) throw std::invalid_argument("goicp: cube rotation index out of range");
	ensure_batch(B, K);
	std::memcpy(h_rots_, rots9, sizeof(Rot9) * K);
	if (cubes != h_cubes_) std::memcpy(h_cubes_, cubes, sizeof(CubeRec) * B);
	HIPCHK(hipMemcpyAsync(d_rots_, h_rots_, sizeof(Rot9) * K, hipMemcpyHostToDevice, stream_));
	HIPCHK(hipMemcpyAsync(d_cubes_, h_cubes_, sizeof(CubeRec) * B, hipMemcpyHostToDevice, stream_));
	bool grouped = false;
	if (B >= 256 && K <= 16 && inliers_ >= (int)N_) {
		size_t sib = 0;
		for (size_t g = 0; g + 8 <= B; g += 8) {
			const CubeRec* c = h_cubes_ + g;
			bool s = true;
			for (int j = 1; j < 8 && s; j++)
// ... 1945 lines not shown
```

cuda-go-icp_amd/csrc/engine.hpp:

```cpp
#pragma once
#include <atomic>
#include <cstdint>
#include <functional>
#include <mutex>
#include <queue>
#include <stdexcept>
#include <string>
#include <vector>

#include "device.hpp"
#include "hipbuf.hpp"

struct goicp_comm_ops;
struct goicp_pose_info_options;
struct goicp_pose_info;

namespace goicp {

struct StatusError : std::runtime_error {
	int rc;
	StatusError(int code, const std::string& msg) : std::runtime_error(msg), rc(code) {}
};

struct IcpShardStats {
	int rank = 0, world = 1;
	int block_begin = 0, block_end = 0, blocks = 0;
	int sliced = 0;
	long long queries = 0, runs = 0, passes = 0, collectives = 0;
	double sum_wait_ms = 0, round_trip_ms = 0;
};

struct Params {
	int dt_size = 300;
	double dt_expand = 2.0;
	float mse_threshold = 1e-3f;
	int dt_layout = 1;
	int device = -1;
	int trans_batch = 32;
	int wide_children = 1;
	int rot_batch = 64;
	int icp_max_iter = 10000;
	int verbose = 0;
	int morton_sort = 2;
	int icp_chunk = 16;
	int kd_gpu_build = -1;
	int bounds_fp16 = 0;
	int icp_nn_cache = 0;
	int flow = 0;
	int adaptive_k = 1;
	int queue_cap = 0;
	int device_queues = 1;
	int icp_point_seed = 1;
	int ub_tiebreak = 0;
	float ub_share = 0.f;
	int sort_items = 1;
	int bounds_order = 2;
	int bounds_order_min_groups = 1024;
	int bounds_order_max_runs = 16;
	float bounds_order_cell = 4.f;
	int bounds_order_reprobe = 64;
	int bounds_balance = 1;
	float bounds_balance_a = 0.f;
	int twin_fusion = 1;
	int lds_tiles = 2;
	float tile_spread_vox = 10.f;
	int stale_widen = 1;
	int stale_compact = 2048;
	int tile_min = 8;
	int lanes = 0;
	int lane_min_searches = 64;
	int stream_priority = 0;
	int icp_fused = 0;
	float trim_fraction = 0.f;
	int use_rot_range = 0, use_trans_range = 0;
	float rot_min[3] = {-180.f, -180.f, -180.f}, rot_max[3] = {180.f, 180.f, 180.f};
	float trans_min[3] = {-0.5f, -0.5f, -0.5f}, trans_max[3] = {0.5f, 0.5f, 0.5f};
	int rot_search_depth = 0, trans_search_depth = 0;
};

struct Counters {
	long long rot_pops = 0, trans_pops = 0, cubes = 0, inner_calls = 0, icp_runs = 0, icp_iters = 0;
	long long bounds_launches = 0;
	long long queue_fallbacks = 0;
	long long tile_expansions = 0;
	long long lane_batches = 0;
};

struct Result {
	float optR[9], optT[3], curR[9], curT[3];
	float best_sse;
	int finished;
	Counters counters;
	double dt_build_ms, register_ms;
};

struct Node {
	float x, y, z, w, ub, lb;
	int l;
	float tie = 0.f;
	friend bool operator<(const Node& a, const Node& b)
	{
		if (a.lb != b.lb) return a.lb > b.lb;
		if (a.w != b.w) return a.w < b.w;
		return a.tie > b.tie;
	}
};

struct StepStatus {
	int finished;
	int early_exit;
	float best_sse;
	float frontier_lb;
	long long rot_pops;
};

class Engine {
public:
	Engine(const Params& p, const float* target_xyz, size_t M, const float* source_xyz, size_t N);
	~Engine();
	Engine(const Engine&) = delete;

	void eval_bounds(const float R[9], const float* cubes4, size_t B, int level, float* ub, float* lb);
	void eval_bounds_batch(const float* rots9, size_t K, const CubeRec* cubes, size_t B, float* ub, float* lb);
	void eval_bounds_dev(const Rot9* d_rots, const CubeRec* d_cubes, int B, float* d_ub, float* d_lb, hipStream_t s, const ParentRec* d_parents = nullptr);
	void reduce_min_dev(const float* d_v, int n, float* d_min, int* d_idx, hipStream_t s);
	float time_bounds_dev(const Rot9* d_rots, const CubeRec* d_cubes, int B, float* d_ub, float* d_lb, int iters, int grouped_nrots = 0);
	void eval_bounds_dev_grouped(const Rot9* d_rots, int nrots, const CubeRec* d_cubes, int B, float* d_ub, float* d_lb, hipStream_t s);
	float eval_sse(const float R[9], const float t[3]);
	float inner_bnb(const float R[9], int level, float incumbent, float best_node[4], Counters* c);
	float icp_run(float R[9], float t[3], int max_iter, float err_diff, int* iters);
	void icp_run_batch(size_t K, float* R, float* t, int max_iter, float err_diff, float* err, int32_t* iters);
	int icp_run_collective(const goicp_comm_ops* comm, float R[9], float t[3], int max_iter, float err_diff, float* err, int* iters);
	const IcpShardStats& icp_shard_stats() const { return icp_shard_; }
	void set_collective_icp(const goicp_comm_ops* comm) { icp_comm_ = comm; unrefined_ = false; }
	bool pose_unrefined() const { return unrefined_; }
	float refine_collective(float R[9], float t[3]);
	float time_icp_pass(const float R[9], const float t[3], int iters, bool cached = false);
	void nn_query(const float* q_xyz, size_t n, int32_t* idx, float* d2);
	void set_icp_options(int metric, int normal_k);
	int icp_metric() const { return icp_metric_; }
	void set_icp_symmetric(int enabled, int source_normal_k);
	bool icp_symmetric() const { return icp_symmetric_; }
	int source_normal_k() const { return source_normal_k_; }
	bool user_source_normals() const { return src_normals_user_; }
	void check_symmetric_query(const char* fn) const;
	void set_icp_generalized(int enabled, float epsilon, int source_normal_k);
	bool icp_generalized() const { return icp_generalized_; }
	float gicp_epsilon() const { return gicp_eps_; }
	void source_normals(float* normals_xyz);
	void set_source_normals(const float* normals_xyz, size_t n);
	void set_icp_gate(float max_corr_dist, int min_inliers, int capped_walk);
	bool icp_gated() const { return gate_dist_ > 0.f; }
	void set_icp_robust(int kernel, float scale);
	void set_search_truncation(float g);
	float search_truncation() const { return dt_.trunc; }
	bool icp_robust() const { return robust_kernel_ != 0; }
	void icp_robust_stats(size_t K, float* cost, float* weight_sum) const;
	void icp_inliers(size_t K, int32_t* out) const;
	void eval_correspondences(const float R[9], const float t[3], float max_corr_dist, int32_t* index, float* dist_sq, int32_t* inliers, float* sse);
	void pose_information(size_t K, const float* R, const float* t, const goicp_pose_info_options* opt, goicp_pose_info* out, bool batch);
	void result_information(const goicp_pose_info_options* opt, goicp_pose_info* out);
	static constexpr double kPoseInfoRankTol = kIcpRankTol;
	void knn_query(const float* q_xyz, size_t n, int k, int32_t* idx, float* d2);
	double normal_build_ms() const { return normal_build_ms_; }
	double source_normal_build_ms() const { return source_normal_build_ms_; }
	void target_normals(float* normals_xyz);
	void icp_step();
	double probe_gather(int mode, size_t window_bytes);
	long long debug_cache_hits(const float R[9], const float t[3]);
	void debug_select(const float* d2, size_t n, int num, int kernel, unsigned char* include);
	void debug_bounds_order(int info[3]);
	void debug_bounds_twins(int info[2]);
	void debug_bounds_balance(int info[26]);
	bool debug_bounds_xcd_spans(unsigned long long* out);
	void debug_queue_expand(const float R[9], int level, const float* parents4, int n, float* ub0, float* lb0, float* ub1, float* lb1, int info[2]);
	struct QueueDigest {
		float* nodes;
		int* counts;
		float* listed;
		float* search;
	};
	void debug_queue_expand_tiles(const float R[9], int level, const float* parents4, int n, int n_ub, float* ub0, float* lb0, float* ub1, float* lb1, int info[4],
	                              const QueueDigest* dg);
	void debug_bounds_tile(const float* rots9, const float* parents4, int nseg, int n, int level, int chunks, float* ub_tile, float* lb_tile,
	                       float* ub_direct, float* lb_direct, float ms[2], unsigned stats[2]);

	void run();
	void cancel() { cancel_.store(true); }
	Result poll();
	void set_progress_callback(std::function<void(const Result&)> cb) { progress_cb_ = std::move(cb); }
	void set_shard(int rank, int world) { rank_ = rank; world_ = world; }
	void register_begin();
	StepStatus register_step(int max_rot_pops);
	void offer_global_best(float sse, const float R[9], const float t[3]);
	void register_end();
	int queue_size() const { return (early_exit_ || converged_) ? 0 : (int)queue_.size(); }
	int donate(int max_nodes, float* nodes7);
	void receive(const float* nodes7, int n);

	const DtDesc& dt() const { return dt_; }
	void dt_download(float* grid_linear);
	size_t n_source() const { return N_; }
	size_t n_target() const { return M_; }
	const float* target_xyz() const { return h_target_.data(); }
	float sse_threshold() const { return sse_thresh_; }
	int device() const { return dev_; }
	int inliers() const { return inliers_; }
	float rot_coeff(int level) const;
	hipStream_t stream() const { return stream_; }
	const float4* d_source() const { return d_src_.get(); }
	void source_transformed(const float R[9], const float t[3], float* out_xyz);
	void set_source(const float* source_xyz, size_t N, const char* fn = "goicp_set_source");
	struct SourceStages {
		float voxel = 0.f;
		int32_t stat_neighbors = 0;
		float stat_std_ratio = 0.f;
		float radius = 0.f;
		int32_t min_neighbors = 0;
		float cluster_radius = 0.f;
		int32_t cluster_min_neighbors = 0, cluster_min_size = 0, cluster_max_clusters = 0;
		float plane_distance = 0.f;
		int32_t plane_iterations = 0, plane_refine = 0, plane_max = 0, plane_min_inliers = 0;
		uint64_t plane_seed = 0;
	};
	void set_source_staged(const char* fn, const float* xyz, size_t n, const SourceStages& st, size_t* n_kept);
	void debug_source_order(const float* xyz, size_t n, int mode, int32_t* perm);
	double last_source_order_ms() const { return source_order_ms_; }
	void voxel_downsample(const float* xyz, size_t n, float voxel, float* out_xyz, int32_t* out_count, size_t* m);
	void radius_outlier_removal(const float* xyz, size_t n, float radius, int32_t min_neighbors, float* out_xyz, int32_t* out_index, int32_t* out_count,
	                            size_t* m);
	void statistical_outlier_removal(const float* xyz, size_t n, int32_t neighbors, float std_ratio, float* out_xyz, int32_t* out_index,
	                                 float* out_mean_dist, double* threshold, size_t* m);
	void knn_self(const float* xyz, size_t n, int32_t k, int32_t* out_index, float* out_dist_sq);
	void estimate_normals(const float* xyz, size_t n, int32_t k, const float* vp, float* out_normals, float* out_variation, int32_t* out_index);
	void fpfh(const float* xyz, const float* normals, size_t n, int32_t k, float* out_fpfh, uint8_t* out_spfh_counts);
	void match_features(const float* q, size_t nq, const float* t, size_t nt, int32_t* out_index, float* out_d2, float* out_d2_second, uint8_t* out_mutual);
	void cluster(const float* xyz, size_t n, float radius, int32_t min_neighbors, int32_t* out_label, int32_t* out_sizes, size_t* n_clusters);
	void cluster_filter(const float* xyz, size_t n, float radius, int32_t min_neighbors, int32_t min_size, int32_t max_clusters, float* out_xyz,
	                    int32_t* out_index, int32_t* out_label, size_t* m);
	void segment_plane(const float* xyz, size_t n, const PlaneSelect& s, int32_t* out_label, PlaneRecord* out_planes, size_t* n_planes);
	void plane_filter(const float* xyz, size_t n, const PlaneSelect& s, float* out_xyz, int32_t* out_index, PlaneRecord* out_planes, size_t* n_planes, size_t* m);
	void ransac_pose(const float* src, size_t n_s, const float* tgt, size_t n_t, const int32_t* corr, size_t M, const RansacPoseSelect& s,
	                 RansacPoseRecord* out_poses, size_t* n_poses, uint8_t* out_inlier);

private:
	Engine(const Params& p, size_t M, size_t N);
	struct InnerSearch;
	void init(const float* target_xyz, size_t M, const float* source_xyz, size_t N);
	static void check_source(const float* source_xyz, size_t N);
	void load_source(const float* source_xyz, size_t N, bool device_order, const float* d_xyz_ready = nullptr);
	void finish_source_swap();
	void sync_lane_streams();
	double source_order_ms_ = 0;
	void ensure_batch(size_t B, size_t K);
	void ensure_stage(size_t B);
// ... 267 lines not shown
```

cuda-go-icp_amd/csrc/goicp_api.cpp:

```cpp
#include "../../include/goicp_mi355.h"

#include <climits>
#include <cstring>
#include <memory>
#include <new>
#include <string>
#include <thread>
#include <vector>

#include "comm.hpp"
#include "config_io.hpp"
#include "engine.hpp"

struct goicp_engine {
	goicp::Engine* e;
};

namespace {

thread_local std::string g_err;

int fail(int code, const std::string& msg)
{
	g_err = msg;
// ... 3 lines not shown
template <class F> int guarded(F&& f)
{
	try {
		f();
		return GOICP_OK;
	} catch (const goicp::StatusError& e) { return fail(e.rc, e.what());
	} catch (const goicp::ConfigError& e) { return fail(GOICP_ERR_CONFIG, e.what());
	} catch (const goicp::IoError& e) { return fail(GOICP_ERR_IO, e.what());
	} catch (const std::invalid_argument& e) { return fail(GOICP_ERR_INVALID, e.what());
	} catch (const std::bad_alloc&) { return fail(GOICP_ERR_INTERNAL, "out of host memory");
	} catch (const std::runtime_error& e) {
		std::string m = e.what();
		return fail(m.find("no HIP device") != std::string::npos ? GOICP_ERR_NO_DEVICE : GOICP_ERR_DEVICE, m);
	} catch (const std::exception& e) { return fail(GOICP_ERR_INTERNAL, e.what());
	} catch (...) { return fail(GOICP_ERR_INTERNAL, "unknown error"); }
}

#define REQUIRE(c) do { if (!(c)) return fail(GOICP_ERR_INVALID, std::string(__func__) + ": invalid argument (" #c ")"); } while (0)

void fill_counters(goicp_counters* o, const goicp::Counters& c)
{
	o->rot_pops = c.rot_pops; o->trans_pops = c.trans_pops; o->cubes = c.cubes; o->inner_calls = c.inner_calls;
	o->icp_runs = c.icp_runs; o->icp_iters = c.icp_iters; o->bounds_launches = c.bounds_launches; o->queue_fallbacks = c.queue_fallbacks;
	o->tile_expansions = c.tile_expansions; o->lane_batches = c.lane_batches;
}

void fill_result(goicp_result* out, const goicp::Result& r)
{
	std::memcpy(out->optR, r.optR, sizeof(r.optR)); std::memcpy(out->optT, r.optT, sizeof(r.optT));
	std::memcpy(out->curR, r.curR, sizeof(r.curR)); std::memcpy(out->curT, r.curT, sizeof(r.curT));
	out->best_sse = r.best_sse; out->finished = r.finished;
	fill_counters(&out->counters, r.counters);
	out->dt_build_ms = r.dt_build_ms; out->register_ms = r.register_ms;
}

}

extern "C" {

const char* goicp_last_error(void) { return g_err.c_str(); }
int goicp_abi_version(void) { return GOICP_ABI_VERSION; }
#ifndef GOICP_KERNEL_HASH
#define GOICP_KERNEL_HASH "unknown"
#endif
const char* goicp_kernel_source_hash(void) { return GOICP_KERNEL_HASH; }

int goicp_config_load(const char* toml_path, goicp_config* out)
{
	REQUIRE(toml_path && out);
	return guarded([&] { goicp::load_config(toml_path, out); });
}

int goicp_cloud_load(const char* path, float subsample, float resize, uint64_t seed, float** xyz, size_t* n)
{
	REQUIRE(path && xyz && n);
	*xyz = nullptr; *n = 0;
	return guarded([&] {
		std::vector<float> v;
		goicp::load_cloud(path, subsample, resize, seed, v);
		float* p = new float[v.size() ? v.size() : 1];
		std::memcpy(p, v.data(), v.size() * sizeof(float));
		*xyz = p; *n = v.size() / 3;
	});
}

void goicp_cloud_free(float* xyz) { delete[] xyz; }

void goicp_params_default(goicp_params* p)
{
	if (!p) return;
	goicp::Params d;
	p->dt_size = d.dt_size; p->dt_expand = d.dt_expand; p->mse_threshold = d.mse_threshold; p->dt_layout = d.dt_layout;
	p->device = d.device; p->trans_batch = d.trans_batch; p->wide_children = d.wide_children;
	p->icp_max_iter = d.icp_max_iter; p->verbose = d.verbose; p->morton_sort = d.morton_sort; p->rot_batch = d.rot_batch; p->trim_fraction = d.trim_fraction; p->kd_gpu_build = d.kd_gpu_build;
	p->use_rot_range = d.use_rot_range; p->use_trans_range = d.use_trans_range;
	for (int k = 0; k < 3; k++) {
		p->rot_min[k] = d.rot_min[k]; p->rot_max[k] = d.rot_max[k];
		p->trans_min[k] = d.trans_min[k]; p->trans_max[k] = d.trans_max[k];
	}
	p->rot_search_depth = d.rot_search_depth; p->trans_search_depth = d.trans_search_depth;
	p->icp_fused = d.icp_fused; p->bounds_fp16 = d.bounds_fp16; p->icp_nn_cache = d.icp_nn_cache; p->flow = d.flow; p->adaptive_k = d.adaptive_k; p->queue_cap = d.queue_cap; p->device_queues = d.device_queues;
	p->lds_tiles = d.lds_tiles; p->tile_spread_vox = d.tile_spread_vox; p->tile_min = d.tile_min; p->stale_widen = d.stale_widen; p->ub_tiebreak = d.ub_tiebreak; p->icp_point_seed = d.icp_point_seed; p->ub_share = d.ub_share; p->twin_fusion = d.twin_fusion; p->sort_items = d.sort_items; p->stale_compact = d.stale_compact; p->stream_priority = d.stream_priority; p->lanes = d.lanes; p->lane_min_searches = d.lane_min_searches;
	p->bounds_order = d.bounds_order; p->bounds_order_min_groups = d.bounds_order_min_groups; p->bounds_order_max_runs = d.bounds_order_max_runs; p->bounds_order_cell = d.bounds_order_cell; p->bounds_order_reprobe = d.bounds_order_reprobe;
	p->bounds_balance = d.bounds_balance; p->bounds_balance_a = d.bounds_balance_a;
}

void goicp_params_from_config(const goicp_config* c, goicp_params* p)
{
	if (!p) return;
	goicp_params_default(p);
	if (!c) return;
	p->mse_threshold = c->mse_threshold;
	if (c->has_rotation_range) {
		p->use_rot_range = 1;
		for (int k = 0; k < 3; k++) { p->rot_min[k] = c->rot_min[k]; p->rot_max[k] = c->rot_max[k]; }
		p->rot_search_depth = c->rot_search_depth;
	}
	if (c->has_translation_range) {
		p->use_trans_range = 1;
		for (int k = 0; k < 3; k++) { p->trans_min[k] = c->trans_min[k]; p->trans_max[k] = c->trans_max[k]; }
		p->trans_search_depth = c->trans_search_depth;
	}
}

int goicp_create(const goicp_params* params, const float* target_xyz, size_t n_target, const float* source_xyz,
                 size_t n_source, goicp_handle* out)
{
	REQUIRE(out);
	*out = nullptr;
	REQUIRE(target_xyz && source_xyz && n_target > 0 && n_source > 0);
	return guarded([&] {
		goicp::Params p;
		if (params) {
			p.dt_size = params->dt_size; p.dt_expand = params->dt_expand; p.mse_threshold = params->mse_threshold;
			p.dt_layout = params->dt_layout; p.device = params->device; p.trans_batch = params->trans_batch;
			p.wide_children = params->wide_children; p.icp_max_iter = params->icp_max_iter; p.verbose = params->verbose;
			p.morton_sort = params->morton_sort;
			if (params->rot_batch > 0) p.rot_batch = params->rot_batch;
			p.trim_fraction = params->trim_fraction;
			p.kd_gpu_build = params->kd_gpu_build;
			p.use_rot_range = params->use_rot_range; p.use_trans_range = params->use_trans_range;
			for (int k = 0; k < 3; k++) {
				p.rot_min[k] = params->rot_min[k]; p.rot_max[k] = params->rot_max[k];
				p.trans_min[k] = params->trans_min[k]; p.trans_max[k] = params->trans_max[k];
			}
			p.rot_search_depth = params->rot_search_depth; p.trans_search_depth = params->trans_search_depth;
			p.icp_fused = params->icp_fused; p.bounds_fp16 = params->bounds_fp16; p.icp_nn_cache = params->icp_nn_cache; p.flow = params->flow; p.adaptive_k = params->adaptive_k; p.queue_cap = params->queue_cap; p.device_queues = params->device_queues;
			p.lds_tiles = params->lds_tiles; p.stale_widen = params->stale_widen; p.ub_tiebreak = params->ub_tiebreak; p.icp_point_seed = params->icp_point_seed; p.ub_share = params->ub_share; p.twin_fusion = params->twin_fusion; p.sort_items = params->sort_items; p.stale_compact = params->stale_compact; p.stream_priority = params->stream_priority; p.lanes = params->lanes; p.lane_min_searches = params->lane_min_searches;
			p.bounds_order = params->bounds_order; p.bounds_order_min_groups = params->bounds_order_min_groups; p.bounds_order_max_runs = params->bounds_order_max_runs; p.bounds_order_reprobe = params->bounds_order_reprobe;
			p.bounds_balance = params->bounds_balance; p.bounds_balance_a = params->bounds_balance_a;
			if (params->bounds_order_cell > 0.f) p.bounds_order_cell = params->bounds_order_cell;
			if (params->tile_spread_vox > 0.f) p.tile_spread_vox = params->tile_spread_vox;
			if (params->tile_min > 0) p.tile_min = params->tile_min;
		}
		goicp_engine* h = new goicp_engine{nullptr};
		try { h->e = new goicp::Engine(p, target_xyz, n_target, source_xyz, n_source); }
		catch (...) { delete h; throw; }
		*out = h;
	});
}

int goicp_destroy(goicp_handle h)
{
	if (!h) return GOICP_OK;
	return guarded([&] { delete h->e; delete h; });
}

int goicp_set_source(goicp_handle h, const float* source_xyz, size_t n_source)
{
	REQUIRE(h && source_xyz && n_source > 0);
	return guarded([&] { h->e->set_source(source_xyz, n_source); });
}

int goicp_source_order_host(const float* xyz, size_t n, int32_t mode, int32_t* perm)
{
	REQUIRE(xyz && perm && n > 0 && mode >= 0 && mode <= 2);
	REQUIRE(n <= (size_t)INT32_MAX / 8);
	return guarded([&] { goicp::source_order_host(xyz, n, mode, perm); });
}

int goicp_debug_source_order(goicp_handle h, const float* xyz, size_t n, int32_t mode, int32_t* perm)
{
	REQUIRE(h && xyz && perm && n > 0);
	return guarded([&] { h->e->debug_source_order(xyz, n, mode, perm); });
}

int goicp_voxel_downsample_host(const float* xyz, size_t n, float voxel, float* out_xyz, int32_t* out_count, size_t* m)
{
	REQUIRE(xyz && out_xyz && m && n > 0);
	REQUIRE(n <= (size_t)INT32_MAX / 8);
	return guarded([&] { goicp::voxel_downsample_host(xyz, n, voxel, out_xyz, out_count, m); });
}

int goicp_voxel_downsample(goicp_handle h, const float* xyz, size_t n, float voxel, float* out_xyz, int32_t* out_count, size_t* m)
{
	REQUIRE(h && xyz && out_xyz && m && n > 0);
	return guarded([&] { h->e->voxel_downsample(xyz, n, voxel, out_xyz, out_count, m); });
}

int goicp_set_source_voxel(goicp_handle h, const float* xyz, size_t n, float voxel, size_t* n_kept)
{
	REQUIRE(h && xyz && n > 0 && voxel != 0.f);
	goicp::Engine::SourceStages st;
	st.voxel = voxel;
	return guarded([&] { h->e->set_source_staged("goicp_set_source_voxel", xyz, n, st, n_kept); });
}

int goicp_radius_outlier_removal_host(const float* xyz, size_t n, float radius, int32_t min_neighbors, float* out_xyz, int32_t* out_index,
                                      int32_t* out_count, size_t* m)
{
	REQUIRE(xyz && out_xyz && m && n > 0);
	REQUIRE(n <= (size_t)INT32_MAX / 8);
	return guarded([&] { goicp::radius_outlier_removal_host(xyz, n, radius, min_neighbors, out_xyz, out_index, out_count, m); });
}

int goicp_radius_outlier_removal(goicp_handle h, const float* xyz, size_t n, float radius, int32_t min_neighbors, float* out_xyz, int32_t* out_index,
                                 int32_t* out_count, size_t* m)
{
	REQUIRE(h && xyz && out_xyz && m && n > 0);
	return guarded([&] { h->e->radius_outlier_removal(xyz, n, radius, min_neighbors, out_xyz, out_index, out_count, m); });
}

void goicp_source_filter_default(goicp_source_filter* out)
{
	if (!out) return;
	out->voxel = 0.f;
	out->radius = 0.f;
	out->min_neighbors = 0;
}

int goicp_set_source_filtered(goicp_handle h, const float* xyz, size_t n, const goicp_source_filter* f, size_t* n_kept)
{
	REQUIRE(h && xyz && f && n > 0);
// ... 286 lines not shown
}

int goicp_device(goicp_handle h, int32_t* ordinal)
{
	REQUIRE(h && ordinal);
	*ordinal = h->e->device();
	return GOICP_OK;
}

int goicp_set_progress_callback(goicp_handle h, goicp_progress_fn cb, void* user)
{
	REQUIRE(h);
	if (!cb) { h->e->set_progress_callback(nullptr); return GOICP_OK; }
	h->e->set_progress_callback([cb, user](const goicp::Result& r) {
		goicp_result out;
		fill_result(&out, r);
		cb(&out, user);
	});
	return GOICP_OK;
}

int goicp_probe_gather(goicp_handle h, int32_t mode, size_t window_bytes, double* lookups_per_s)
{
	REQUIRE(h && lookups_per_s && (mode == 0 || mode == 1 || mode == 2 || mode == 4 || mode == 8 || mode == 16 || mode == 32));
	return guarded([&] { *lookups_per_s = h->e->probe_gather(mode, window_bytes); });
}

int goicp_debug_cache_hits(goicp_handle h, const float R[9], const float t[3], int64_t* hits)
{
	REQUIRE(h && R && t && hits);
	return guarded([&] { *hits = h->e->debug_cache_hits(R, t); });
}

int goicp_debug_bounds_tile(goicp_handle h, const float* rots9, const float* parents4, int32_t nseg, int32_t n, int32_t level, int32_t chunks,
                            float* ub_tile, float* lb_tile, float* ub_direct, float* lb_direct, float ms[2], uint32_t stats[2])
{
	REQUIRE(h && rots9 && parents4 && ub_tile && lb_tile && ub_direct && lb_direct && ms && stats);
	return guarded([&] { h->e->debug_bounds_tile(rots9, parents4, nseg, n, level, chunks, ub_tile, lb_tile, ub_direct, lb_direct, ms, stats); });
}

int goicp_debug_queue_expand(goicp_handle h, const float R[9], int32_t level, const float* parents4, int32_t n, float* ub_ubpass, float* lb_ubpass,
                             float* ub_lbpass, float* lb_lbpass, int32_t info[2])
{
	REQUIRE(h && R && parents4 && ub_ubpass && lb_ubpass && ub_lbpass && lb_lbpass && info && n >= 1);
	return guarded([&] {
		int inf[2] = {0, 0};
		h->e->debug_queue_expand(R, level, parents4, n, ub_ubpass, lb_ubpass, ub_lbpass, lb_lbpass, inf);
		info[0] = inf[0]; info[1] = inf[1];
	});
}

int goicp_debug_queue_expand_tiles(goicp_handle h, const float R[9], int32_t level, const float* parents4, int32_t n, int32_t n_ub, float* ub_ubpass,
                                   float* lb_ubpass, float* ub_lbpass, float* lb_lbpass, int32_t info[4], int32_t digest, float* queue_nodes,
                                   int32_t* queue_counts, float* listed4, float* search8)
{
	REQUIRE(h && R && parents4 && ub_ubpass && lb_ubpass && ub_lbpass && lb_lbpass && info && n >= 1 && n_ub >= 1 && n_ub <= n);
	REQUIRE(!digest || (queue_nodes && queue_counts && listed4 && search8));
	return guarded([&] {
		int inf[4] = {0, 0, 0, 0}, counts[4] = {0, 0, 0, 0};
		const goicp::Engine::QueueDigest dg{queue_nodes, counts, listed4, search8};
		h->e->debug_queue_expand_tiles(R, level, parents4, n, n_ub, ub_ubpass, lb_ubpass, ub_lbpass, lb_lbpass, inf, digest ? &dg : nullptr);
		for (int k = 0; k < 4; k++) info[k] = inf[k];
		if (digest) for (int k = 0; k < 4; k++) queue_counts[k] = counts[k];
	});
}

int goicp_debug_bounds_order(goicp_handle h, int32_t info[3])
{
	REQUIRE(h && info);
	return guarded([&] {
		int inf[3] = {0, 0, 0};
		h->e->debug_bounds_order(inf);
		info[0] = inf[0]; info[1] = inf[1]; info[2] = inf[2];
	});
}

int goicp_debug_bounds_twins(goicp_handle h, int32_t info[2])
{
	REQUIRE(h && info);
	return guarded([&] {
		int inf[2] = {0, 0};
		h->e->debug_bounds_twins(inf);
		info[0] = inf[0]; info[1] = inf[1];
	});
}

int goicp_debug_bounds_balance(goicp_handle h, int32_t info[26])
{
	REQUIRE(h && info);
	return guarded([&] {
		int inf[26];
		h->e->debug_bounds_balance(inf);
		for (int k = 0; k < 26; k++) info[k] = inf[k];
	});
}

int goicp_debug_bounds_xcd_spans(goicp_handle h, uint64_t out[96])
{
	REQUIRE(h && out);
	static_assert(goicp::kXcdStampRows * goicp::kXcdStampCols == 96, "goicp_debug_bounds_xcd_spans: 96 words");
	return guarded([&] {
		unsigned long long w[96];
		if (!h->e->debug_bounds_xcd_spans(w)) throw std::invalid_argument("goicp_debug_bounds_xcd_spans: not a diagnostic build (GOICP_BOUNDS_XCD_STAMPS)");
		for (int k = 0; k < 96; k++) out[k] = w[k];
	});
}

int goicp_debug_select(goicp_handle h, const float* d2, size_t n, int32_t num, int32_t kernel, uint8_t* include)
{
	REQUIRE(h && d2 && include && n >= 1 && n <= 0x7fffffffu && num >= 1 && (size_t)num <= n && kernel >= 0 && kernel <= 2 && !(kernel == 1 && n > 32768));
	return guarded([&] { h->e->debug_select(d2, n, num, kernel, include); });
}

int goicp_debug_kabsch(const float H[9], float R[9])
{
	REQUIRE(H && R);
	return guarded([&] { goicp::debug_kabsch(H, R); });
}

int goicp_dt_info(goicp_handle h, int32_t* V, double* scale, double origin[3])
{
	REQUIRE(h);
	const goicp::DtDesc& d = h->e->dt();
	if (V) *V = d.V;
	if (scale) *scale = d.scale;
	if (origin) { origin[0] = d.xmin; origin[1] = d.ymin; origin[2] = d.zmin; }
	return GOICP_OK;
}

int goicp_dt_download(goicp_handle h, float* grid)
{
	REQUIRE(h && grid);
	return guarded([&] { h->e->dt_download(grid); });
}

int goicp_eval_bounds(goicp_handle h, const float R[9], const float* cubes, size_t B, int32_t level, float* ub, float* lb)
{
	REQUIRE(h && R && (B == 0 || (cubes && ub && lb)));
	return guarded([&] { h->e->eval_bounds(R, cubes, B, level, ub, lb); });
}

int goicp_eval_bounds_batch(goicp_handle h, const float* rots, size_t K, const goicp_cube* cubes, size_t B, float* ub, float* lb)
{
	REQUIRE(h && (B == 0 || (rots && K > 0 && cubes && ub && lb)));
	static_assert(sizeof(goicp_cube) == sizeof(goicp::CubeRec), "goicp_cube layout");
	return guarded([&] { h->e->eval_bounds_batch(rots, K, reinterpret_cast<const goicp::CubeRec*>(cubes), B, ub, lb); });
}

int goicp_eval_bounds_device(goicp_handle h, const void* d_rots, const void* d_cubes, size_t B, void* d_ub, void* d_lb, void* stream)
{
	REQUIRE(h && d_rots && d_cubes && d_ub && d_lb && B > 0);
	return guarded([&] {
		h->e->eval_bounds_dev(static_cast<const goicp::Rot9*>(d_rots), static_cast<const goicp::CubeRec*>(d_cubes), (int)B,
		                      static_cast<float*>(d_ub), static_cast<float*>(d_lb), static_cast<hipStream_t>(stream));
	});
}

int goicp_eval_bounds_device_grouped(goicp_handle h, const void* d_rots, size_t n_rots, const void* d_cubes, size_t B, void* d_ub, void* d_lb, void* stream)
{
	REQUIRE(h && d_rots && d_cubes && d_ub && d_lb && B > 0 && n_rots >= 1 && n_rots <= 16);
	return guarded([&] {
		h->e->eval_bounds_dev_grouped(static_cast<const goicp::Rot9*>(d_rots), (int)n_rots, static_cast<const goicp::CubeRec*>(d_cubes), (int)B,
		                              static_cast<float*>(d_ub), static_cast<float*>(d_lb), static_cast<hipStream_t>(stream));
	});
}

// ... 568 lines not shown
```

include/goicp_mi355.h:

```cpp
#ifndef GOICP_MI355_H
#define GOICP_MI355_H

#include <stddef.h>
#include <stdint.h>

#ifdef __cplusplus
extern "C" {
#endif

#define GOICP_ABI_VERSION 4

typedef enum goicp_status {
	GOICP_OK = 0,
	GOICP_ERR_INVALID = -1,
	GOICP_ERR_IO = -2,
	GOICP_ERR_CONFIG = -3,
	GOICP_ERR_NO_DEVICE = -4,
	GOICP_ERR_DEVICE = -5,
	GOICP_ERR_INTERNAL = -6,
	GOICP_ERR_TIMEOUT = -7,
	GOICP_ERR_PEER = -8
} goicp_status;

const char* goicp_last_error(void);
int goicp_abi_version(void);
const char* goicp_kernel_source_hash(void);

#define GOICP_PATH_MAX 1024
typedef struct goicp_config {
	int32_t mode;
	int32_t trim;
	float subsample;
	float mse_threshold;
	float resize;
	char target[GOICP_PATH_MAX];
	char source[GOICP_PATH_MAX];
	char output[GOICP_PATH_MAX];
	char visualization[GOICP_PATH_MAX];
	float viz_theta, viz_phi;
	int32_t viz_spin_after_finish;
	float rot_min[3], rot_max[3];
	int32_t rot_search_depth;
	float trans_min[3], trans_max[3];
	int32_t trans_search_depth;
	char description[GOICP_PATH_MAX];
	int32_t has_rotation_range;
	int32_t has_translation_range;
} goicp_config;

int goicp_config_load(const char* toml_path, goicp_config* out);

int goicp_cloud_load(const char* path, float subsample, float resize, uint64_t seed, float** xyz, size_t* n);
void goicp_cloud_free(float* xyz);

typedef struct goicp_engine* goicp_handle;

typedef struct goicp_params {
	int32_t dt_size;
	double dt_expand;
	float mse_threshold;
	int32_t dt_layout;
	int32_t device;
	int32_t trans_batch;
	int32_t wide_children;
	int32_t icp_max_iter;
	int32_t verbose;
	int32_t morton_sort;
	int32_t rot_batch;
	int32_t kd_gpu_build;
	float trim_fraction;
	int32_t use_rot_range, use_trans_range;
	float rot_min[3], rot_max[3];
	float trans_min[3], trans_max[3];
	int32_t rot_search_depth, trans_search_depth;
	int32_t icp_fused;
	int32_t bounds_fp16;
	int32_t icp_nn_cache;
	int32_t flow;
	int32_t adaptive_k;
	int32_t queue_cap;
	int32_t device_queues;
	int32_t lds_tiles;
	float tile_spread_vox;
	int32_t tile_min;
	int32_t stale_widen;
	int32_t ub_tiebreak;
	int32_t icp_point_seed;
	float ub_share;
	int32_t twin_fusion;
	int32_t sort_items;
	int32_t stale_compact;
	int32_t stream_priority;
	int32_t lanes;
	int32_t lane_min_searches;
	int32_t bounds_order;
	int32_t bounds_order_min_groups;
	int32_t bounds_order_max_runs;
	float bounds_order_cell;
	int32_t bounds_order_reprobe;
	int32_t bounds_balance;
	float bounds_balance_a;
} goicp_params;

void goicp_params_default(goicp_params* p);
void goicp_params_from_config(const goicp_config* c, goicp_params* p);

int goicp_create(const goicp_params* params, const float* target_xyz, size_t n_target,
                 const float* source_xyz, size_t n_source, goicp_handle* out);
int goicp_destroy(goicp_handle h);
int goicp_set_source(goicp_handle h, const float* source_xyz, size_t n_source);
int goicp_source_order_host(const float* xyz, size_t n, int32_t mode, int32_t* perm);
int goicp_voxel_downsample_host(const float* xyz, size_t n, float voxel, float* out_xyz, int32_t* out_count, size_t* m);
int goicp_voxel_downsample(goicp_handle h, const float* xyz, size_t n, float voxel, float* out_xyz, int32_t* out_count, size_t* m);
int goicp_set_source_voxel(goicp_handle h, const float* xyz, size_t n, float voxel, size_t* n_kept);
int goicp_radius_outlier_removal_host(const float* xyz, size_t n, float radius, int32_t min_neighbors, float* out_xyz, int32_t* out_index, int32_t* out_count, size_t* m);
int goicp_radius_outlier_removal(goicp_handle h, const float* xyz, size_t n, float radius, int32_t min_neighbors, float* out_xyz, int32_t* out_index, int32_t* out_count, size_t* m);
typedef struct goicp_source_filter { float voxel; float radius; int32_t min_neighbors; } goicp_source_filter;
void goicp_source_filter_default(goicp_source_filter* out);
int goicp_set_source_filtered(goicp_handle h, const float* xyz, size_t n, const goicp_source_filter* f, size_t* n_kept);
#define GOICP_STAT_MAX_NEIGHBORS 64
int goicp_statistical_outlier_removal_host(const float* xyz, size_t n, int32_t neighbors, float std_ratio, float* out_xyz, int32_t* out_index, float* out_mean_dist, double* threshold, size_t* m);
int goicp_statistical_outlier_removal(goicp_handle h, const float* xyz, size_t n, int32_t neighbors, float std_ratio, float* out_xyz, int32_t* out_index, float* out_mean_dist, double* threshold, size_t* m);
typedef struct goicp_source_pipeline { float voxel; int32_t stat_neighbors; float stat_std_ratio; float radius; int32_t min_neighbors; } goicp_source_pipeline;
void goicp_source_pipeline_default(goicp_source_pipeline* out);
int goicp_set_source_pipeline(goicp_handle h, const float* xyz, size_t n, const goicp_source_pipeline* p, size_t* n_kept);
#define GOICP_KNN_SELF_MAX 32
int goicp_knn_self_host(const float* xyz, size_t n, int32_t k, int32_t* out_index, float* out_dist_sq);
int goicp_knn_self(goicp_handle h, const float* xyz, size_t n, int32_t k, int32_t* out_index, float* out_dist_sq);
int goicp_estimate_normals_host(const float* xyz, size_t n, int32_t k, const float vp[3], float* out_normals, float* out_variation, int32_t* out_index);
int goicp_estimate_normals(goicp_handle h, const float* xyz, size_t n, int32_t k, const float vp[3], float* out_normals, float* out_variation, int32_t* out_index);
#define GOICP_FPFH_DIM 33
#define GOICP_FPFH_COS { 0x1.aeb8c8764f0bap-1, 0x1.a9628d9c712b6p-2, -0x1.2375f640f44dbp-3, -0x1.4f49e7f775887p-1, -0x1.eb42a9bcd5057p-1, \
                         -0x1.eb42a9bcd5057p-1, -0x1.4f49e7f775887p-1, -0x1.2375f640f44dbp-3, 0x1.a9628d9c712b6p-2, 0x1.aeb8c8764f0bap-1 }
#define GOICP_FPFH_SIN { 0x1.14cedf8bb580bp-1, 0x1.d1bb48eee2c13p-1, 0x1.fac9e043842efp-1, 0x1.82f19bb3a28a1p-1, 0x1.207e7fd768dbfp-2, \
                         -0x1.207e7fd768dbfp-2, -0x1.82f19bb3a28a1p-1, -0x1.fac9e043842efp-1, -0x1.d1bb48eee2c13p-1, -0x1.14cedf8bb580bp-1 }
int goicp_fpfh_host(const float* xyz, const float* normals, size_t n, int32_t k, float* out_fpfh, uint8_t* out_spfh_counts);
int goicp_fpfh(goicp_handle h, const float* xyz, const float* normals, size_t n, int32_t k, float* out_fpfh, uint8_t* out_spfh_counts);
int goicp_match_features_host(const float* query, size_t n_q, const float* target, size_t n_t, int32_t* out_index, float* out_d2, float* out_d2_second,
                              uint8_t* out_mutual);
int goicp_match_features(goicp_handle h, const float* query, size_t n_q, const float* target, size_t n_t, int32_t* out_index, float* out_d2,
                         float* out_d2_second, uint8_t* out_mutual);
int goicp_match_features_tile(void);
int goicp_cluster_host(const float* xyz, size_t n, float radius, int32_t min_neighbors, int32_t* out_label, int32_t* out_sizes, size_t* n_clusters);
int goicp_cluster(goicp_handle h, const float* xyz, size_t n, float radius, int32_t min_neighbors, int32_t* out_label, int32_t* out_sizes, size_t* n_clusters);
typedef struct goicp_cluster_select { float radius; int32_t min_neighbors; int32_t min_size; int32_t max_clusters; } goicp_cluster_select;
void goicp_cluster_select_default(goicp_cluster_select* out);
int goicp_cluster_filter_host(const float* xyz, size_t n, const goicp_cluster_select* s, float* out_xyz, int32_t* out_index, int32_t* out_label, size_t* m);
int goicp_cluster_filter(goicp_handle h, const float* xyz, size_t n, const goicp_cluster_select* s, float* out_xyz, int32_t* out_index, int32_t* out_label, size_t* m);
int goicp_set_source_clustered(goicp_handle h, const float* xyz, size_t n, const goicp_source_pipeline* p, const goicp_cluster_select* s, size_t* n_kept);
#define GOICP_PLANE_MAX_ITERATIONS 65536
#define GOICP_PLANE_MAX_PLANES 8
typedef struct goicp_plane_select {
    float    distance;
    int32_t  iterations;
    int32_t  refine;
    int32_t  max_planes;
    int32_t  min_inliers;
    uint64_t seed;
} goicp_plane_select;
typedef struct goicp_plane {
    float   normal[3];
    float   point[3];
    float   d;
    int32_t inliers;
    int32_t hypothesis;
    int32_t refined;
} goicp_plane;
void goicp_plane_select_default(goicp_plane_select* out);
int goicp_segment_plane_host(const float* xyz, size_t n, const goicp_plane_select* sel, int32_t* out_label, goicp_plane* out_planes, size_t* n_planes);
int goicp_segment_plane(goicp_handle h, const float* xyz, size_t n, const goicp_plane_select* sel, int32_t* out_label, goicp_plane* out_planes, size_t* n_planes);
int goicp_plane_filter_host(const float* xyz, size_t n, const goicp_plane_select* sel, float* out_xyz, int32_t* out_index, goicp_plane* out_planes,
                            size_t* n_planes, size_t* m);
int goicp_plane_filter(goicp_handle h, const float* xyz, size_t n, const goicp_plane_select* sel, float* out_xyz, int32_t* out_index, goicp_plane* out_planes,
                       size_t* n_planes, size_t* m);
int goicp_set_source_segmented(goicp_handle h, const float* xyz, size_t n, const goicp_source_pipeline* p, const goicp_plane_select* pl,
                               const goicp_cluster_select* s, size_t* n_kept);
#define GOICP_RANSAC_POSE_MAX_ITERATIONS (1 << 20)
#define GOICP_RANSAC_POSE_MAX_POSES 64
typedef struct goicp_ransac_pose_select {
    float    distance;
    int32_t  iterations;
    int32_t  refine;
    int32_t  max_poses;
    int32_t  min_inliers;
// ... 154 lines not shown
int goicp_set_shard(goicp_handle h, int32_t rank, int32_t world);
int goicp_register_begin(goicp_handle h);
int goicp_register_step(goicp_handle h, int32_t max_rot_pops, goicp_step_status* out);
int goicp_offer_best(goicp_handle h, float sse, const float R[9], const float t[3]);
int goicp_register_end(goicp_handle h);

typedef struct goicp_comm_ops {
	void* ctx;
	int32_t rank, world;
	int (*allreduce_min_u64)(void* ctx, uint64_t* words, size_t n);
	int (*bcast)(void* ctx, void* buf, size_t bytes, int32_t root);
} goicp_comm_ops;
typedef struct goicp_shard_stats {
	int64_t steps, exchanges, broadcasts, donations, donated_cubes;
	int64_t steps_idle;
	double wait_ms;
	double step_ms;
	float best_sse;
	int32_t failed_rank;
} goicp_shard_stats;
typedef struct goicp_shard_options {
	int32_t rot_pops_per_step;
	int32_t rebalance;
	int32_t stale_exchange;
	int32_t ramp_to;
} goicp_shard_options;
typedef struct goicp_shard_engine_ops {
	void* ctx;
	float sse_threshold;
	int (*begin)(void* ctx, int32_t rank, int32_t world);
	int (*step)(void* ctx, int32_t max_rot_pops, goicp_step_status* out);
	int (*pose)(void* ctx, float* sse, float R[9], float t[3]);
	int (*offer)(void* ctx, float sse, const float R[9], const float t[3]);
	int (*queue_size)(void* ctx, int32_t* n);
	int (*donate)(void* ctx, int32_t max_nodes, float* nodes7, int32_t* n);
	int (*receive)(void* ctx, const float* nodes7, int32_t n);
	int (*end)(void* ctx);
} goicp_shard_engine_ops;
int goicp_run_sharded(const goicp_shard_engine_ops* engine, const goicp_comm_ops* comm, int32_t rot_pops_per_step,
                      int32_t rebalance, goicp_shard_stats* stats);
int goicp_register_sharded(goicp_handle h, const goicp_comm_ops* comm, int32_t rot_pops_per_step, int32_t rebalance,
                           goicp_shard_stats* stats);
void goicp_shard_options_default(goicp_shard_options* out);
int goicp_run_sharded_opt(const goicp_shard_engine_ops* engine, const goicp_comm_ops* comm, const goicp_shard_options* opt,
                          goicp_shard_stats* stats);
int goicp_register_sharded_opt(goicp_handle h, const goicp_comm_ops* comm, const goicp_shard_options* opt, goicp_shard_stats* stats);
int goicp_comm_allreduce_sum_i64(const goicp_comm_ops* comm, int64_t* words, size_t n);
int goicp_icp_run_collective(goicp_handle h, const goicp_comm_ops* comm, float R[9], float t[3], int32_t max_iter, float err_diff,
                             float* err, int32_t* iters);
typedef struct goicp_icp_shard_stats {
	int32_t rank, world;
	int32_t block_begin, block_end;
	int32_t blocks;
	int32_t sliced;
	int64_t queries;
	int64_t runs, passes, collectives;
	double sum_wait_ms;
	double round_trip_ms;
} goicp_icp_shard_stats;
int goicp_icp_shard_stats_get(goicp_handle h, goicp_icp_shard_stats* out);
int goicp_register_sharded_collective_icp(goicp_handle h, const goicp_comm_ops* comm, const goicp_shard_options* opt, goicp_shard_stats* stats);
int goicp_comm_set_timeout_ms(goicp_comm_ops* comm, int32_t timeout_ms);
int goicp_thread_comm_create(int32_t world, goicp_comm_ops* out );
int goicp_thread_comm_destroy(goicp_comm_ops* comm);
#define GOICP_RCCL_ID_BYTES 128
int goicp_rccl_unique_id(char id128[GOICP_RCCL_ID_BYTES]);
int goicp_rccl_comm_create(const char id128[GOICP_RCCL_ID_BYTES], int32_t rank, int32_t world, int32_t device, goicp_comm_ops* out);
int goicp_rccl_comm_wrap(void* nccl_comm, int32_t rank, int32_t world, int32_t device, goicp_comm_ops* out);
int goicp_rccl_comm_destroy(goicp_comm_ops* comm);
int goicp_register_multi_gpu(const goicp_params* params, const float* target_xyz, size_t n_target, const float* source_xyz,
                             size_t n_source, int32_t world, int32_t rot_pops_per_step, goicp_handle* out, goicp_shard_stats* stats);

int goicp_probe_gather(goicp_handle h, int32_t mode, size_t window_bytes, double* lookups_per_s);
int goicp_debug_kabsch(const float H[9], float R[9]);
int goicp_debug_bounds_tile(goicp_handle h, const float* rots9, const float* parents4, int32_t nseg, int32_t n, int32_t level, int32_t chunks,
                            float* ub_tile, float* lb_tile, float* ub_direct, float* lb_direct, float ms[2], uint32_t stats[2]);
int goicp_debug_queue_expand(goicp_handle h, const float R[9], int32_t level, const float* parents4, int32_t n, float* ub_ubpass, float* lb_ubpass,
                             float* ub_lbpass, float* lb_lbpass, int32_t info[2]);
int goicp_debug_queue_expand_tiles(goicp_handle h, const float R[9], int32_t level, const float* parents4, int32_t n, int32_t n_ub, float* ub_ubpass,
                                   float* lb_ubpass, float* ub_lbpass, float* lb_lbpass, int32_t info[4], int32_t digest, float* queue_nodes,
                                   int32_t* queue_counts, float* listed4, float* search8);
int goicp_debug_bounds_order(goicp_handle h, int32_t info[3]);
int goicp_debug_bounds_twins(goicp_handle h, int32_t info[2]);
int goicp_debug_bounds_balance(goicp_handle h, int32_t info[26]);
int goicp_debug_bounds_xcd_spans(goicp_handle h, uint64_t out[96]);
int goicp_debug_cache_hits(goicp_handle h, const float R[9], const float t[3], int64_t* hits);
int goicp_debug_select(goicp_handle h, const float* d2, size_t n, int32_t num, int32_t kernel, uint8_t* include);
int goicp_debug_source_order(goicp_handle h, const float* xyz, size_t n, int32_t mode, int32_t* perm);

#ifdef __cplusplus
}
#endif
#endif
```

Before: 46.04 million cube-bounds/s.

## Deduplicate identical cube groups in pair bounds kernel via LDS hash aliasing

Adds a hash-table pass in the bounds order kernel that detects cube groups with byte-identical records within a run and records an alias to the first owner. The pair bounds kernel then skips computing bounds for alias copies, and the finalize kernel reads the owner's scratch rows. This removes redundant DT lookups for duplicate cubes in a batch, at the cost of an extra hashing pass with LDS atomics, a full record compare per hit, and extra indirection in finalize. It is enabled by default through a new bounds_dedup parameter.

```diff
diff --git a/cuda-go-icp_amd/binding.py b/cuda-go-icp_amd/binding.py
--- a/cuda-go-icp_amd/binding.py
+++ b/cuda-go-icp_amd/binding.py
@@ -37,7 +37,7 @@
                 ("icp_fused", C.c_int32), ("bounds_fp16", C.c_int32), ("icp_nn_cache", C.c_int32), ("flow", C.c_int32), ("adaptive_k", C.c_int32), ("queue_cap", C.c_int32), ("device_queues", C.c_int32),
                 ("lds_tiles", C.c_int32), ("tile_spread_vox", C.c_float), ("tile_min", C.c_int32), ("stale_widen", C.c_int32), ("ub_tiebreak", C.c_int32), ("icp_point_seed", C.c_int32), ("ub_share", C.c_float), ("twin_fusion", C.c_int32), ("sort_items", C.c_int32), ("stale_compact", C.c_int32), ("stream_priority", C.c_int32), ("lanes", C.c_int32), ("lane_min_searches", C.c_int32),
                 ("bounds_order", C.c_int32), ("bounds_order_min_groups", C.c_int32), ("bounds_order_max_runs", C.c_int32), ("bounds_order_cell", C.c_float), ("bounds_order_reprobe", C.c_int32),
-                ("bounds_balance", C.c_int32), ("bounds_balance_a", C.c_float)]
+                ("bounds_balance", C.c_int32), ("bounds_balance_a", C.c_float), ("bounds_dedup", C.c_int32)]
 
 
 class CCube(C.Structure):
@@ -183,6 +183,7 @@
     "goicp_debug_cache_hits": (C.c_int, [_vp, _fp, _fp, C.POINTER(C.c_int64)]),
     "goicp_debug_bounds_order": (C.c_int, [_vp, C.POINTER(C.c_int32)]),
     "goicp_debug_bounds_twins": (C.c_int, [_vp, C.POINTER(C.c_int32)]),
+    "goicp_debug_bounds_copies": (C.c_int, [_vp, C.POINTER(C.c_int32)]),
     "goicp_debug_bounds_balance": (C.c_int, [_vp, C.POINTER(C.c_int32)]),
     "goicp_debug_bounds_xcd_spans": (C.c_int, [_vp, C.POINTER(C.c_uint64)]),
     "goicp_debug_select": (C.c_int, [_vp, _fp, C.c_size_t, C.c_int32, C.c_int32, C.POINTER(C.c_uint8)]),
diff --git a/cuda-go-icp_amd/csrc/device.hip b/cuda-go-icp_amd/csrc/device.hip
--- a/cuda-go-icp_amd/csrc/device.hip
+++ b/cuda-go-icp_amd/csrc/device.hip
@@ -800,7 +800,8 @@
 	}
 }
 
-__global__ void bounds_finalize(const float* __restrict__ scratch, int B, int groups, int chunks, float* __restrict__ ub_out, float* __restrict__ lb_out);
+__global__ void bounds_finalize(const float* __restrict__ scratch, int B, int groups, int chunks, float* __restrict__ ub_out, float* __restrict__ lb_out,
+                                const int* __restrict__ alias, const int* __restrict__ ctl);
 hipError_t launch_bounds_tile(const float4* src, int N, const DtDesc& dt, const Rot9* rots, const ParentRec* parents, const void* segs, int nseg, int n,
                               int chunks, float* scratch, float* ub, float* lb, unsigned* stats, hipStream_t stream)
 {
@@ -811,7 +812,7 @@
 	                   static_cast<const TileSeg*>(segs), nseg, chunks, cp, static_cast<const int*>(nullptr), static_cast<int*>(nullptr), scratch, ub, lb, stats);
 	if (chunks > 1) {
 		const int groups = nseg * n, t = groups * 2 * kGroup;
-		hipLaunchKernelGGL(bounds_finalize, dim3((t + 255) / 256), dim3(256), 0, stream, scratch, groups * kGroup, groups, chunks, ub, lb);
+		hipLaunchKernelGGL(bounds_finalize, dim3((t + 255) / 256), dim3(256), 0, stream, scratch, groups * kGroup, groups, chunks, ub, lb, (const int*)nullptr, (const int*)nullptr);
 	}
 	return hipGetLastError();
 }
@@ -965,6 +966,25 @@
 	}
 	return key;
 }
+__device__ __forceinline__ unsigned alias_hash(const CubeRec& a, const CubeRec& b)
+{
+	const unsigned w[12] = {__float_as_uint(a.tx), __float_as_uint(a.ty), __float_as_uint(a.tz), __float_as_uint(a.delta), __float_as_uint(a.coeff), (unsigned)a.rot,
+	                        __float_as_uint(b.tx), __float_as_uint(b.ty), __float_as_uint(b.tz), __float_as_uint(b.delta), __float_as_uint(b.coeff), (unsigned)b.rot};
+	unsigned h = 0x9e3779b9u;
+#pragma unroll
+	for (int k = 0; k < 12; k++) { h = (h ^ w[k]) * 0x85ebca6bu; h ^= h >> 15; }
+	return h;
+}
+__device__ __forceinline__ bool same_records(const CubeRec* __restrict__ cubes, int ga, int gb)
+{
+	constexpr int nw = kGroup * (int)(sizeof(CubeRec) / sizeof(unsigned));
+	const unsigned* a = reinterpret_cast<const unsigned*>(cubes + (size_t)ga * kGroup);
+	const unsigned* b = reinterpret_cast<const unsigned*>(cubes + (size_t)gb * kGroup);
+	unsigned d = 0u;
+#pragma unroll
+	for (int k = 0; k < nw; k++) d |= a[k] ^ b[k];
+	return d == 0u;
+}
 constexpr int kOrderHeld = 4;
 __device__ __forceinline__ void bounds_cuts_store(const BoundsOrder& bo, int balanced, int items, int lane)
 {
@@ -1011,7 +1031,7 @@
 	const int nb = nbound, runs = nb + 1;
 	if (runs > bo.max_runs) {
 		if (blockIdx.x == 0 && tid == 0) {
-			bo.ctl[0] = 0; bo.ctl[1] = 0; bo.ctl[2] = 0; bo.ctl[3] = 0; if (bo.host_note) *bo.host_note = ((long long)G << 1) | 1;
+			bo.ctl[0] = 0; bo.ctl[1] = 0; bo.ctl[2] = 0; bo.ctl[3] = 0; bo.ctl[kBoundsCopies] = 0; if (bo.host_note) *bo.host_note = ((long long)G << 1) | 1;
 		}
 		if (blockIdx.x == 0 && tid < 64) bounds_cuts_store(bo, balanced, (G + 1) >> 1, tid);
 		return;
@@ -1029,7 +1049,7 @@
 	const int s0 = run_start[run], n = run_start[run + 1] - s0;
 	int item0 = 0, items = 0;
 	for (int q = 0; q < runs; q++) { if (q == run) item0 = items; items += (run_start[q + 1] - run_start[q] + 1) >> 1; }
-	if (run == 0 && tid == 0) { bo.ctl[0] = items; bo.ctl[1] = 1; bo.ctl[2] = 0; bo.ctl[3] = 0; if (bo.host_note) *bo.host_note = (long long)G << 1; }
+	if (run == 0 && tid == 0) { bo.ctl[0] = items; bo.ctl[1] = 1; bo.ctl[2] = 0; bo.ctl[3] = 0; bo.ctl[kBoundsCopies] = 0; if (bo.host_note) *bo.host_note = (long long)G << 1; }
 	if (run == 0 && tid < 64) bounds_cuts_store(bo, balanced, items, tid);
 	float held[kOrderHeld][3];
 	float lo[3] = {INFINITY, INFINITY, INFINITY}, hi[3] = {-INFINITY, -INFINITY, -INFINITY};
@@ -1102,6 +1122,29 @@
 		float c[3];
 		group_centre(cubes, s0 + j, B, c);
 		place(order_key(c, lo, to_cell), j);
+	}
+	if (!bo.alias) return;
+	__syncthreads();
+	unsigned long long* table = reinterpret_cast<unsigned long long*>(lds);
+	int slots = 64;
+	while (slots < 2 * n && slots < kSortBins / 2) slots <<= 1;
+	for (int i = tid; i < slots / 2; i += 1024) reinterpret_cast<uint4*>(lds)[i] = make_uint4(~0u, ~0u, ~0u, ~0u);
+	__syncthreads();
+	for (int j = tid; j < n; j += 1024) {
+		const int g = s0 + j;
+		int owner = g;
+		if (g * kGroup + kGroup <= B) {
+			const unsigned h = alias_hash(cubes[(size_t)g * kGroup], cubes[(size_t)g * kGroup + kGroup - 1]);
+			const unsigned long long mine = ((unsigned long long)h << 32) | (unsigned)j;
+			unsigned slot = h & (unsigned)(slots - 1);
+			for (int probe = 0; probe < kBoundsAliasProbes; probe++) {
+				const unsigned long long old = atomicCAS(&table[slot], ~0ull, mine);
+				if (old == ~0ull) break;
+				if ((unsigned)(old >> 32) == h && same_records(cubes, g, s0 + (int)(unsigned)old)) { owner = s0 + (int)(unsigned)old; break; }
+				slot = (slot + 1) & (unsigned)(slots - 1);
+			}
+		}
+		bo.alias[g] = owner;
 	}
 }
 
@@ -1152,7 +1195,8 @@
 GOICP_BOUNDS_PAIR_HEAD(
     const float4* __restrict__ src, int N, DtDesc dt, const Rot9* __restrict__ rots,
     const CubeRec* __restrict__ cubes, const ParentRec* __restrict__ parents, int B, int groups, int max_items, int chunks, int chunk_pts,
-    float* __restrict__ scratch, float* __restrict__ ub_out, float* __restrict__ lb_out, const int* __restrict__ pairs, int* __restrict__ ctl)
+    float* __restrict__ scratch, float* __restrict__ ub_out, float* __restrict__ lb_out, const int* __restrict__ pairs, int* __restrict__ ctl,
+    const int* __restrict__ alias)
 {
 	__shared__ float red[kBoundsThreads / 64][2 * kGroup];
 	const int work = blockIdx.x, total = gridDim.x;
@@ -1181,17 +1225,24 @@
 		if (ga >= groups) return;
 		gb = ga + 1 < groups ? ga + 1 : -1;
 	}
+	int copy = 0;
+	if (listed && alias && chunks > 1) {
+		copy = (alias[ga] != ga ? 1 : 0) | (gb >= 0 && alias[gb] != gb ? 2 : 0);
+		if (copy && chunk == 0 && threadIdx.x == 0) atomicAdd(ctl + kBoundsCopies, (copy & 1) + (copy >> 1));
+	}
 	if (listed && gb >= 0) {
 		PairMember A, Bm;
 		int ra, rb;
 		const bool sa = pair_member(cubes, parents, ga, B, A, ra), sb = pair_member(cubes, parents, gb, B, Bm, rb);
-		if (sa && sb && ra == rb) {
+		const bool both = sa && sb && ra == rb;
+		if (both && chunk == 0 && threadIdx.x == 0 && same_box(A, Bm))
+			atomicAdd(ctl + (__float_as_uint(A.coeff) == __float_as_uint(Bm.coeff) || (A.coeff == 0.f && Bm.coeff == 0.f) ? 3 : 2), 1);
+		if (both && !copy) {
 			const Rot9 R0 = rots[ra];
 			const int p0 = chunk * chunk_pts;
 			const int p1 = p0 + chunk_pts < N ? p0 + chunk_pts : N;
 			if (same_box(A, Bm)) {
 				const bool same = __float_as_uint(A.coeff) == __float_as_uint(Bm.coeff) || (A.coeff == 0.f && Bm.coeff == 0.f);
-				if (chunk == 0 && threadIdx.x == 0) atomicAdd(ctl + (same ? 3 : 2), 1);
 				float ub[kGroup], lb[kGroup];
 				if (same) {
 					f2 ub2[1][4], lb2[1][4];
@@ -1256,6 +1307,8 @@
 			if (bad != 3) gb = -1;
 		}
 	}
+	if (copy & 2) gb = -1;
+	if (copy & 1) { ga = gb; gb = -1; }
 #pragma unroll 1
 	for (int m = 0; m < 2; m++) {
 		const int g = m ? gb : ga;
@@ -1272,10 +1325,11 @@
 __global__ __launch_bounds__(kBoundsThreads) void bounds_pair_kernel(
     const float4* __restrict__ src, int N, DtDesc dt, const Rot9* __restrict__ rots,
     const CubeRec* __restrict__ cubes, const ParentRec* __restrict__ parents, int B, int groups, int max_items, int chunks, int chunk_pts,
-    float* __restrict__ scratch, float* __restrict__ ub_out, float* __restrict__ lb_out, const int* __restrict__ pairs, int* __restrict__ ctl)
+    float* __restrict__ scratch, float* __restrict__ ub_out, float* __restrict__ lb_out, const int* __restrict__ pairs, int* __restrict__ ctl,
+    const int* __restrict__ alias)
 {
 	const unsigned long long t0 = wall_clock64();
-	bounds_pair_body<TRUNC>(src, N, dt, rots, cubes, parents, B, groups, max_items, chunks, chunk_pts, scratch, ub_out, lb_out, pairs, ctl);
+	bounds_pair_body<TRUNC>(src, N, dt, rots, cubes, parents, B, groups, max_items, chunks, chunk_pts, scratch, ub_out, lb_out, pairs, ctl, alias);
 	__syncthreads();
 	if (threadIdx.x == 0) {
 		const unsigned long long t1 = wall_clock64();
@@ -1329,14 +1383,15 @@
 }
 
 __global__ void bounds_finalize(const float* __restrict__ scratch, int B, int groups, int chunks,
-                                float* __restrict__ ub_out, float* __restrict__ lb_out)
+                                float* __restrict__ ub_out, float* __restrict__ lb_out, const int* __restrict__ alias, const int* __restrict__ ctl)
 {
 	int t = blockIdx.x * blockDim.x + threadIdx.x;
 	if (t >= groups * 2 * kGroup) return;
 	int group = t / (2 * kGroup), k = t - group * 2 * kGroup;
 	int c = group * kGroup + (k & (kGroup - 1));
 	if (c >= B) return;
-	const float* s = scratch + (size_t)group * chunks * (2 * kGroup) + k;
+	const int rows = alias && ctl[1] ? alias[group] : group;
+	const float* s = scratch + (size_t)rows * chunks * (2 * kGroup) + k;
 	float acc = 0.f;
 	for (int j = 0; j < chunks; j++) acc += s[(size_t)j * 2 * kGroup];
 	(k < kGroup ? ub_out : lb_out)[c] = acc;
@@ -1694,9 +1749,14 @@
 	int groups, chunks, chunk_pts;
 	bounds_shape(B, N, &groups, &chunks, &chunk_pts);
 	dim3 grid(groups * chunks), block(kBoundsThreads);
+	const int* alias = nullptr;
+	const int* alias_ctl = nullptr;
 	if (bo && bo->mode > 0 && cubes && !parents && dt.layout == 1 && bounds_lean(dt) && groups >= bo->min_groups && bo->max_runs >= 1 && bo->max_runs <= kBoundsOrderMaxRuns) {
 		const bool balanced = bo->mode == 2 && chunks == 8 && bo->balance && bo->cost;
-		hipLaunchKernelGGL(bounds_order_kernel, dim3(bo->max_runs), dim3(1024), 0, stream, cubes, B, groups, dt, *bo, balanced ? 1 : 0);
+		BoundsOrder pre = *bo;
+		if (bo->mode != 2 || chunks == 1) pre.alias = nullptr;
+		alias = pre.alias; alias_ctl = pre.alias ? bo->ctl : nullptr;
+		hipLaunchKernelGGL(bounds_order_kernel, dim3(bo->max_runs), dim3(1024), 0, stream, cubes, B, groups, dt, pre, balanced ? 1 : 0);
 		if (bo->mode == 1) {
 			hipLaunchKernelGGL((dt.trunc > 0.f ? bounds_ordered_kernel<true> : bounds_ordered_kernel<false>), grid, block, 0, stream, src, N, dt, rots, cubes, parents, B, groups,
 			                   chunks, chunk_pts, scratch, ub, lb, bo->order, bo->ctl, 1);
@@ -1704,7 +1764,7 @@
 			const int max_items = (int)bounds_order_items(groups, bo->max_runs);
 			const int nblocks = chunks == 8 ? 8 * bounds_pair_slots(max_items, balanced) : max_items * chunks;
 			hipLaunchKernelGGL((dt.trunc > 0.f ? bounds_pair_kernel<true> : bounds_pair_kernel<false>), dim3(nblocks), block, 0, stream, src, N, dt, rots, cubes, parents,
-			                   B, groups, max_items, chunks, chunk_pts, scratch, ub, lb, bo->pairs, bo->ctl);
+			                   B, groups, max_items, chunks, chunk_pts, scratch, ub, lb, bo->pairs, bo->ctl, alias);
 		}
 	} else
 	if (dt.trunc > 0.f) {
@@ -1727,7 +1787,7 @@
 		hipLaunchKernelGGL(bounds_kernel<2>, grid, block, 0, stream, src, N, dt, rots, cubes, parents, B, groups, chunks, chunk_pts, scratch, ub, lb);
 	if (chunks > 1) {
 		int t = groups * 2 * kGroup;
-		hipLaunchKernelGGL(bounds_finalize, dim3((t + 255) / 256), dim3(256), 0, stream, scratch, B, groups, chunks, ub, lb);
+		hipLaunchKernelGGL(bounds_finalize, dim3((t + 255) / 256), dim3(256), 0, stream, scratch, B, groups, chunks, ub, lb, alias, alias_ctl);
 	}
 	return hipGetLastError();
 }
diff --git a/cuda-go-icp_amd/csrc/device.hpp b/cuda-go-icp_amd/csrc/device.hpp
--- a/cuda-go-icp_amd/csrc/device.hpp
+++ b/cuda-go-icp_amd/csrc/device.hpp
@@ -92,7 +92,7 @@
 	int mode;
 	int min_groups, max_runs;
 	float cell_vox;
-	unsigned* keys;
+	int* alias;
 	unsigned* order;
 	int* pairs;
 	int* ctl;
@@ -101,7 +101,8 @@
 	int balance;
 };
 constexpr int kBoundsOrderMaxRuns = 64;
-constexpr int kBoundsCut = 4, kBoundsCtlInts = 32;
+constexpr int kBoundsCut = 4, kBoundsCopies = 13, kBoundsCtlInts = 32;
+constexpr int kBoundsAliasProbes = 32;
 constexpr float kBoundsBalanceA = 18.f;
 inline size_t bounds_order_items(int groups, int max_runs) { return (size_t)(groups + 1) / 2 + (size_t)max_runs; }
 inline int bounds_pair_slots(int max_items, bool balanced) { return balanced ? (int)(((long long)max_items * 5 + 3) / 4) : max_items; }
diff --git a/cuda-go-icp_amd/csrc/engine.cpp b/cuda-go-icp_amd/csrc/engine.cpp
--- a/cuda-go-icp_amd/csrc/engine.cpp
+++ b/cuda-go-icp_amd/csrc/engine.cpp
@@ -1199,8 +1199,8 @@
 	}
 	border_.mode = p_.bounds_order >= 2 ? 2 : 1;
 	border_.min_groups = p_.bounds_order_min_groups; border_.max_runs = max_runs; border_.cell_vox = p_.bounds_order_cell;
-	border_.keys = d_border_.get(); border_.order = border_.keys + groups;
-	border_.pairs = reinterpret_cast<int*>(border_.order + groups); border_.ctl = reinterpret_cast<int*>(border_.keys + ctl_at);
+	border_.alias = p_.bounds_dedup != 0 ? reinterpret_cast<int*>(d_border_.get()) : nullptr; border_.order = d_border_.get() + groups;
+	border_.pairs = reinterpret_cast<int*>(border_.order + groups); border_.ctl = reinterpret_cast<int*>(d_border_.get() + ctl_at);
 	border_.host_note = h_border_note_.get();
 	border_.cost = d_bcost_.get(); border_.balance = p_.bounds_balance != 0;
 	return &border_;
@@ -1242,6 +1242,15 @@
 	if (border_form_ != 2) return;
 	HIPCHK(hipStreamSynchronize(border_stream_));
 	HIPCHK(hipMemcpy(info, border_.ctl + 2, 2 * sizeof(int), hipMemcpyDeviceToHost));
+}
+
+void Engine::debug_bounds_copies(int info[1])
+{
+	DeviceGuard guard(dev_);
+	info[0] = 0;
+	if (border_form_ != 2) return;
+	HIPCHK(hipStreamSynchronize(border_stream_));
+	HIPCHK(hipMemcpy(info, border_.ctl + kBoundsCopies, sizeof(int), hipMemcpyDeviceToHost));
 }
 
 void Engine::debug_bounds_balance(int info[26])
diff --git a/cuda-go-icp_amd/csrc/engine.hpp b/cuda-go-icp_amd/csrc/engine.hpp
--- a/cuda-go-icp_amd/csrc/engine.hpp
+++ b/cuda-go-icp_amd/csrc/engine.hpp
@@ -61,6 +61,7 @@
 	int bounds_order_reprobe = 64;
 	int bounds_balance = 1;
 	float bounds_balance_a = 0.f;
+	int bounds_dedup = 1;
 	int twin_fusion = 1;
 	int lds_tiles = 2;
 	float tile_spread_vox = 10.f;
@@ -171,6 +172,7 @@
 	void debug_select(const float* d2, size_t n, int num, int kernel, unsigned char* include);
 	void debug_bounds_order(int info[3]);
 	void debug_bounds_twins(int info[2]);
+	void debug_bounds_copies(int info[1]);
 	void debug_bounds_balance(int info[26]);
 	bool debug_bounds_xcd_spans(unsigned long long* out);
 	void debug_queue_expand(const float R[9], int level, const float* parents4, int n, float* ub0, float* lb0, float* ub1, float* lb1, int info[2]);
diff --git a/cuda-go-icp_amd/csrc/goicp_api.cpp b/cuda-go-icp_amd/csrc/goicp_api.cpp
--- a/cuda-go-icp_amd/csrc/goicp_api.cpp
+++ b/cuda-go-icp_amd/csrc/goicp_api.cpp
@@ -109,7 +109,7 @@
 	p->icp_fused = d.icp_fused; p->bounds_fp16 = d.bounds_fp16; p->icp_nn_cache = d.icp_nn_cache; p->flow = d.flow; p->adaptive_k = d.adaptive_k; p->queue_cap = d.queue_cap; p->device_queues = d.device_queues;
 	p->lds_tiles = d.lds_tiles; p->tile_spread_vox = d.tile_spread_vox; p->tile_min = d.tile_min; p->stale_widen = d.stale_widen; p->ub_tiebreak = d.ub_tiebreak; p->icp_point_seed = d.icp_point_seed; p->ub_share = d.ub_share; p->twin_fusion = d.twin_fusion; p->sort_items = d.sort_items; p->stale_compact = d.stale_compact; p->stream_priority = d.stream_priority; p->lanes = d.lanes; p->lane_min_searches = d.lane_min_searches;
 	p->bounds_order = d.bounds_order; p->bounds_order_min_groups = d.bounds_order_min_groups; p->bounds_order_max_runs = d.bounds_order_max_runs; p->bounds_order_cell = d.bounds_order_cell; p->bounds_order_reprobe = d.bounds_order_reprobe;
-	p->bounds_balance = d.bounds_balance; p->bounds_balance_a = d.bounds_balance_a;
+	p->bounds_balance = d.bounds_balance; p->bounds_balance_a = d.bounds_balance_a; p->bounds_dedup = d.bounds_dedup;
 }
 
 void goicp_params_from_config(const goicp_config* c, goicp_params* p)
@@ -155,7 +155,7 @@
 			p.icp_fused = params->icp_fused; p.bounds_fp16 = params->bounds_fp16; p.icp_nn_cache = params->icp_nn_cache; p.flow = params->flow; p.adaptive_k = params->adaptive_k; p.queue_cap = params->queue_cap; p.device_queues = params->device_queues;
 			p.lds_tiles = params->lds_tiles; p.stale_widen = params->stale_widen; p.ub_tiebreak = params->ub_tiebreak; p.icp_point_seed = params->icp_point_seed; p.ub_share = params->ub_share; p.twin_fusion = params->twin_fusion; p.sort_items = params->sort_items; p.stale_compact = params->stale_compact; p.stream_priority = params->stream_priority; p.lanes = params->lanes; p.lane_min_searches = params->lane_min_searches;
 			p.bounds_order = params->bounds_order; p.bounds_order_min_groups = params->bounds_order_min_groups; p.bounds_order_max_runs = params->bounds_order_max_runs; p.bounds_order_reprobe = params->bounds_order_reprobe;
-			p.bounds_balance = params->bounds_balance; p.bounds_balance_a = params->bounds_balance_a;
+			p.bounds_balance = params->bounds_balance; p.bounds_balance_a = params->bounds_balance_a; p.bounds_dedup = params->bounds_dedup;
 			if (params->bounds_order_cell > 0.f) p.bounds_order_cell = params->bounds_order_cell;
 			if (params->tile_spread_vox > 0.f) p.tile_spread_vox = params->tile_spread_vox;
 			if (params->tile_min > 0) p.tile_min = params->tile_min;
@@ -608,6 +608,16 @@
 		int inf[2] = {0, 0};
 		h->e->debug_bounds_twins(inf);
 		info[0] = inf[0]; info[1] = inf[1];
+	});
+}
+
+int goicp_debug_bounds_copies(goicp_handle h, int32_t info[1])
+{
+	REQUIRE(h && info);
+	return guarded([&] {
+		int inf[1] = {0};
+		h->e->debug_bounds_copies(inf);
+		info[0] = inf[0];
 	});
 }
 
diff --git a/include/goicp_mi355.h b/include/goicp_mi355.h
--- a/include/goicp_mi355.h
+++ b/include/goicp_mi355.h
@@ -100,6 +100,7 @@
 	int32_t bounds_order_reprobe;
 	int32_t bounds_balance;
 	float bounds_balance_a;
+	int32_t bounds_dedup;
 } goicp_params;
 
 void goicp_params_default(goicp_params* p);
@@ -420,6 +421,7 @@
                                    int32_t* queue_counts, float* listed4, float* search8);
 int goicp_debug_bounds_order(goicp_handle h, int32_t info[3]);
 int goicp_debug_bounds_twins(goicp_handle h, int32_t info[2]);
+int goicp_debug_bounds_copies(goicp_handle h, int32_t info[1]);
 int goicp_debug_bounds_balance(goicp_handle h, int32_t info[26]);
 int goicp_debug_bounds_xcd_spans(goicp_handle h, uint64_t out[96]);
 int goicp_debug_cache_hits(goicp_handle h, const float R[9], const float t[3], int64_t* hits);
```

After: 49.54 million cube-bounds/s, median of 6. +7.6%, better.
